# DLR-RM/curvature

Measured on AMD Instinct MI355X. Metric: KFAC factor-build + invert + sample throughput, higher is better.
Workload: dtype f32

## Files before the change

### curvature_amd/_lib.py

```python
import ctypes
import os
import subprocess
import threading

_HERE = os.path.dirname(os.path.abspath(__file__))
CSRC = os.path.join(_HERE, "csrc")
INCLUDE = os.path.normpath(os.path.join(_HERE, "..", "include"))
LIB_PATH = os.path.join(CSRC, "libcurv_hip.so")
SOURCES = ["api.cpp", "collective.cpp", "elementwise.hip", "syrk.hip", "syrk_flat.hip", "syrk_corr.hip", "syrk_pre.hip", "syrk_small.hip", "group_factor.hip", "kfac_half.hip", "convt_factor.hip", "dilated_factor.hip", "conv3d_factor.hip", "reduce_factor.hip", "persample.hip", "persample_dw.hip", "norm_factor.hip", "logit_mc.hip", "head_mc.hip", "head_grid.hip", "invert.hip", "gemm.hip", "inf.hip", "eigh.hip", "eigh_lowrank.hip", "logdet.hip"]
HIPCC_FLAGS = ["-O3", "--offload-arch=gfx950", "-std=c++17", "-fPIC", "-shared", "-Wall",
               "-Wno-unused-function", "-ldl"]

_lock = threading.Lock()
_lib = None


def _stale() -> bool:
    if not os.path.exists(LIB_PATH):
        return True
    t = os.path.getmtime(LIB_PATH)
    deps = [os.path.join(CSRC, f) for f in os.listdir(CSRC) if f.endswith((".hip", ".cpp", ".h"))]
    deps.append(os.path.join(INCLUDE, "curv_hip.h"))
    return any(os.path.getmtime(d) > t for d in deps)


def _compiler_id(hipcc: str) -> str:
    try:
        return subprocess.run([hipcc, "--version"], stdout=subprocess.PIPE, stderr=subprocess.STDOUT, text=True).stdout
    except OSError as exc:
        raise RuntimeError(f"cannot run {hipcc}: {exc}")


def build(force: bool = False, verbose: bool = False) -> str:
    if not force and not _stale():
        return LIB_PATH
    import fcntl
    import hashlib
    from concurrent.futures import ThreadPoolExecutor
    hipcc = os.environ.get("HIPCC", "hipcc")
    objdir = os.path.join(CSRC, "build")
    os.makedirs(objdir, exist_ok=True)
    headers = sorted([os.path.join(CSRC, f) for f in os.listdir(CSRC) if f.endswith(".h")] + [os.path.join(INCLUDE, "curv_hip.h")])
    compile_flags = [f for f in HIPCC_FLAGS if f not in ("-shared", "-ldl")] + ["-c"]
    base = hashlib.sha256()
    base.update(_compiler_id(hipcc).encode())
    base.update(" ".join(compile_flags).encode())
    for h in headers:
        base.update(open(h, "rb").read())

    def compile_one(src):
        path = os.path.join(CSRC, src)
        obj = os.path.join(objdir, src + ".o")
        key = base.copy()
        key.update(open(path, "rb").read())
        stamp, want = obj + ".stamp", key.hexdigest()
        if not force and os.path.exists(obj) and os.path.exists(stamp) and open(stamp).read() == want:
            return obj, 0, ""
        tmp = f"{obj}.{os.getpid()}.tmp"
        cmd = [hipcc] + compile_flags + ["-o", tmp, path]
        if verbose:
            print(" ".join(cmd[:-3] + ["-o", obj, path]), flush=True)
        proc = subprocess.run(cmd, stdout=subprocess.PIPE, stderr=subprocess.STDOUT, text=True)
        if proc.returncode == 0:
            os.replace(tmp, obj)
            with open(stamp + ".tmp", "w") as fh:
                fh.write(want)
            os.replace(stamp + ".tmp", stamp)
        elif os.path.exists(tmp):
            os.remove(tmp)
        return obj, proc.returncode, proc.stdout

    with open(os.path.join(objdir, ".lock"), "w") as lock:
        fcntl.flock(lock, fcntl.LOCK_EX)
        try:
            if not force and not _stale():
                return LIB_PATH
            with ThreadPoolExecutor(max_workers=int(os.environ.get("CURV_BUILD_JOBS", "6"))) as pool:
                results = list(pool.map(compile_one, SOURCES))
            for obj, rc, out in results:
                if rc != 0:
                    raise RuntimeError("hipcc failed:\n" + out)
                if verbose and out:
                    print(out)
            tmp = f"{LIB_PATH}.{os.getpid()}.tmp"
            cmd = [hipcc, "--offload-arch=gfx950", "-fPIC", "-shared", "-o", tmp] + [r[0] for r in results] + ["-ldl"]
            if verbose:
                print(" ".join(cmd), flush=True)
            proc = subprocess.run(cmd, stdout=subprocess.PIPE, stderr=subprocess.STDOUT, text=True)
            if proc.returncode != 0:
                if os.path.exists(tmp):
                    os.remove(tmp)
                raise RuntimeError("hipcc (link) failed:\n" + proc.stdout)
            os.replace(tmp, LIB_PATH)
        finally:
            fcntl.flock(lock, fcntl.LOCK_UN)
    return LIB_PATH


_ENDS = [("src", ctypes.c_void_p), ("dst", ctypes.c_void_p)]
_SOURCE = [(k, ctypes.c_int32) for k in ("N", "C", "H", "W")]
_WINDOW = [(k, ctypes.c_int32) for k in ("kh", "kw", "sh", "sw", "ph", "pw")]
_ENTRY = [("has_bias", ctypes.c_int32), ("first", ctypes.c_int32), ("scale", ctypes.c_float)]


class curv_factor_desc(ctypes.Structure):
    _fields_ = _ENDS + _SOURCE + _WINDOW + _ENTRY + [("path_hint", ctypes.c_int32)]


class curv_group_factor_desc(ctypes.Structure):
    _fields_ = _ENDS + _SOURCE + [("groups", ctypes.c_int32)] + _WINDOW + _ENTRY


class curv_convt_factor_desc(ctypes.Structure):
    _fields_ = _ENDS + _SOURCE + _WINDOW + [("Ho", ctypes.c_int32), ("Wo", ctypes.c_int32)] + _ENTRY


class curv_dilated_factor_desc(ctypes.Structure):
    _fields_ = _ENDS + _SOURCE + _WINDOW + _ENTRY + [("dh", ctypes.c_int32), ("dw", ctypes.c_int32)]


class curv_conv3d_factor_desc(ctypes.Structure):
    _fields_ = _ENDS + [(k, ctypes.c_int32) for k in ("N", "C", "D", "H", "W", "kd", "kh", "kw", "sd", "sh", "sw", "pd", "ph",
                                                     "pw")] + _ENTRY


class curv_reduce_factor_desc(ctypes.Structure):
    _fields_ = _ENDS + _SOURCE + _WINDOW + _ENTRY + [(k, ctypes.c_int32) for k in ("dtype", "form", "mean", "T", "E")]


class curv_factor16_desc(ctypes.Structure):
    _fields_ = _ENDS + _SOURCE + _WINDOW + _ENTRY + [("dtype", ctypes.c_int32)]


class curv_inv_desc(ctypes.Structure):
    _fields_ = [("F", ctypes.c_void_p), ("L", ctypes.c_void_p), ("n", ctypes.c_int32), ("reserved", ctypes.c_int32),
                ("add", ctypes.c_double), ("multiply", ctypes.c_double)]


class curv_gemm_desc(ctypes.Structure):
    _fields_ = [("A", ctypes.c_void_p), ("B", ctypes.c_void_p), ("C", ctypes.c_void_p), ("E", ctypes.c_void_p)] + \
               [(k, ctypes.c_longlong) for k in ("a_rs", "a_cs", "b_rs", "b_cs", "c_rs", "c_cs", "e_rs", "e_cs")] + \
               [("M", ctypes.c_int32), ("N", ctypes.c_int32), ("K", ctypes.c_int32), ("epilogue", ctypes.c_int32),
                ("alpha", ctypes.c_float), ("beta", ctypes.c_float), ("tri", ctypes.c_int32),
                ("reserved", ctypes.c_int32), ("F", ctypes.c_void_p), ("f_rs", ctypes.c_longlong),
                ("f_cs", ctypes.c_longlong)]


class curv_cholinv_desc(ctypes.Structure):
    _fields_ = [("M", ctypes.c_void_p), ("X", ctypes.c_void_p), ("n", ctypes.c_int32), ("m_is_f64", ctypes.c_int32),
                ("diag_add", ctypes.c_double), ("R", ctypes.c_void_p), ("r_minus", ctypes.c_int32), ("reserved", ctypes.c_int32),
                ("pivot_min", ctypes.c_double)]


class curv_gemm64_desc(ctypes.Structure):
    _fields_ = [("A", ctypes.c_void_p), ("B", ctypes.c_void_p), ("C", ctypes.c_void_p)] + \
               [(k, ctypes.c_longlong) for k in ("a_rs", "a_cs", "b_rs", "b_cs", "c_rs", "c_cs")] + \
               [("M", ctypes.c_int32), ("N", ctypes.c_int32), ("K", ctypes.c_int32), ("tri", ctypes.c_int32),
                ("alpha", ctypes.c_double), ("beta", ctypes.c_double),
                ("E", ctypes.c_void_p), ("row_scale", ctypes.c_void_p), ("col_scale", ctypes.c_void_p), ("C32", ctypes.c_void_p)]


class curv_sq_desc(ctypes.Structure):
    _fields_ = [("grad_w", ctypes.c_void_p), ("grad_b", ctypes.c_void_p), ("state", ctypes.c_void_p),
                ("rows", ctypes.c_int32), ("cols_w", ctypes.c_int32), ("first", ctypes.c_int32),
                ("reserved", ctypes.c_int32)]


class curv_persample_desc(ctypes.Structure):
    _fields_ = [("A", ctypes.c_void_p), ("B", ctypes.c_void_p), ("C", ctypes.c_void_p)] + \
               [(k, ctypes.c_longlong) for k in ("a_ns", "a_rs", "b_ns", "b_rs", "c_rs")] + \
               [("S", ctypes.c_int32), ("M", ctypes.c_int32), ("Nc", ctypes.c_int32), ("L", ctypes.c_int32),
                ("first", ctypes.c_int32), ("alpha", ctypes.c_float)]


class curv_persample_quad_desc(ctypes.Structure):
    _fields_ = [("A", ctypes.c_void_p), ("B", ctypes.c_void_p), ("W", ctypes.c_void_p), ("out", ctypes.c_void_p)] + \
               [(k, ctypes.c_longlong) for k in ("a_ns", "a_rs", "b_ns", "b_rs", "w_rs", "o_stride")] + \
               [("S", ctypes.c_int32), ("M", ctypes.c_int32), ("Nc", ctypes.c_int32), ("L", ctypes.c_int32),
                ("first", ctypes.c_int32), ("alpha", ctypes.c_float)]


class curv_persample_project_desc(ctypes.Structure):
    _fields_ = [(k, ctypes.c_void_p) for k in ("A", "B", "W", "U", "Z")] + \
               [(k, ctypes.c_longlong) for k in ("a_ns", "a_rs", "b_ns", "b_rs", "w_rs", "u_rs", "z_ns", "z_rs", "z_cs")] + \
               [(k, ctypes.c_int32) for k in ("S", "M", "Nc", "L", "R", "first")] + \
               [("alpha", ctypes.c_float), ("reserved", ctypes.c_int32)]


class curv_persample_grid_desc(ctypes.Structure):
    _fields_ = [(k, ctypes.c_void_p) for k in ("A", "B", "u", "v", "V", "out")] + \
               [("shift", ctypes.POINTER(ctypes.c_float)), ("gain", ctypes.POINTER(ctypes.c_float))] + \
               [(k, ctypes.c_longlong) for k in ("a_ns", "a_rs", "b_ns", "b_rs", "v_rs", "o_stride", "o_hs")] + \
               [(k, ctypes.c_int32) for k in ("S", "M", "Nc", "L", "H", "first")]


class curv_persample_cov_desc(ctypes.Structure):
    _fields_ = [("A", ctypes.c_void_p), ("B", ctypes.c_void_p), ("W", ctypes.c_void_p), ("out", ctypes.c_void_p)] + \
               [(k, ctypes.c_longlong) for k in ("a_cs", "a_ns", "a_rs", "b_ns", "b_rs", "w_rs", "o_ns", "o_rs")] + \
               [(k, ctypes.c_int32) for k in ("S", "K", "M", "Nc", "L", "first")] + [("alpha", ctypes.c_float)]


class curv_logit_mc_desc(ctypes.Structure):
    _fields_ = [(k, ctypes.c_void_p) for k in ("cov", "mu", "rest", "Z", "probs", "probs_rest", "draws", "info")] + \
               [(k, ctypes.c_longlong) for k in ("o_ns", "o_rs", "mu_ns", "z_ns", "z_ss")] + \
               [("seed", ctypes.c_ulonglong), ("offset", ctypes.c_ulonglong)] + \
               [(k, ctypes.c_int32) for k in ("N", "K", "S", "reserved")]


class curv_head_mc_desc(ctypes.Structure):
    _fields_ = [(k, ctypes.c_void_p) for k in ("M", "d2", "mu", "Z", "probs", "draws")] + \
               [(k, ctypes.c_longlong) for k in ("m_rs", "d_ns", "d_cs", "mu_ns", "z_ns", "z_ss")] + \
               [("seed", ctypes.c_ulonglong), ("offset", ctypes.c_ulonglong)] + \
               [(k, ctypes.c_int32) for k in ("N", "K", "S", "m_lower")] + [("reserved", ctypes.c_longlong)]


class curv_head_moments_desc(ctypes.Structure):
    _fields_ = curv_head_mc_desc._fields_[:-1] + \
               [("entropy", ctypes.c_void_p), ("probs_sq", ctypes.c_void_p), ("reserved", ctypes.c_longlong)]


class curv_head_grid_desc(ctypes.Structure):
    _fields_ = [(k, ctypes.c_void_p) for k in ("Y", "u", "v", "T", "out")] + \
               [("shift", ctypes.POINTER(ctypes.c_float)), ("gain", ctypes.POINTER(ctypes.c_float))] + \
               [(k, ctypes.c_longlong) for k in ("y_rs", "t_rs")] + [(k, ctypes.c_int32) for k in ("N", "K", "n", "H")]


class curv_persample_pack_desc(ctypes.Structure):
    _fields_ = _ENDS + _SOURCE + _WINDOW + \
               [(k, ctypes.c_int32) for k in ("has_bias", "channels_last", "rows_outer", "Lp")]


class curv_persample_pack_ex_desc(ctypes.Structure):
    _fields_ = _ENDS + [(k, ctypes.c_longlong) for k in ("s_n", "s_c", "s_h", "s_w", "src_elems")] + _SOURCE + _WINDOW + \
               [(k, ctypes.c_int32) for k in ("Ho", "Wo", "has_bias", "dtype", "transposed", "rows_outer", "Lp", "reserved")]


class curv_persample_pack3d_desc(ctypes.Structure):
    _fields_ = _ENDS + [(k, ctypes.c_longlong) for k in ("s_n", "s_c", "s_d", "s_h", "s_w", "src_elems")] + \
               [(k, ctypes.c_int32) for k in ("N", "C", "D", "H", "W", "kd", "kh", "kw", "sd", "sh", "sw", "pd", "ph", "pw",
                                              "has_bias", "dtype", "rows_outer", "Lp", "reserved")]


class curv_persample_dw_desc(ctypes.Structure):
    _fields_ = [("x", ctypes.c_void_p), ("g", ctypes.c_void_p)] + \
               [(k, ctypes.c_longlong) for k in ("x_sn", "x_sc", "x_sh", "x_sw", "x_elems",
                                                 "g_sn", "g_sc", "g_sh", "g_sw", "g_elems")] + _SOURCE + _WINDOW + \
               [(k, ctypes.c_int32) for k in ("Ho", "Wo", "has_bias", "first")] + [("alpha", ctypes.c_float),
                                                                                   ("reserved", ctypes.c_int32)] + \
               [("dst", ctypes.c_void_p), ("c_rs", ctypes.c_longlong)] + \
               [(k, ctypes.c_void_p) for k in ("T", "Wt", "s", "out")] + \
               [(k, ctypes.c_longlong) for k in ("t_cs", "t_rs", "w_rs", "o_stride")]


class curv_norm_desc(ctypes.Structure):
    _fields_ = [("x", ctypes.c_void_p), ("g", ctypes.c_void_p)] + \
               [(k, ctypes.c_longlong) for k in ("x_sn", "x_sc", "x_sh", "x_sw", "x_elems",
                                                 "g_sn", "g_sc", "g_sh", "g_sw", "g_elems")] + _SOURCE + \
               [("mode", ctypes.c_int32), ("groups", ctypes.c_int32), ("eps", ctypes.c_float), ("has_bias", ctypes.c_int32),
                ("mean", ctypes.c_void_p), ("var", ctypes.c_void_p), ("side", ctypes.c_int32), ("first", ctypes.c_int32),
                ("scale", ctypes.c_float), ("alpha", ctypes.c_float), ("reserved", ctypes.c_int32),
                ("reserved2", ctypes.c_int32), ("dst", ctypes.c_void_p), ("c_rs", ctypes.c_longlong)] + \
               [(k, ctypes.c_void_p) for k in ("T", "Wt", "s", "out")] + \
               [(k, ctypes.c_longlong) for k in ("t_cs", "t_rs", "w_rs", "o_stride")]


_DW_RECORD = [("x", ctypes.c_void_p), ("g", ctypes.c_void_p)] + \
             [(k, ctypes.c_longlong) for k in ("x_sn", "x_sc", "x_sh", "x_sw", "x_elems",
                                               "g_sn", "g_sc", "g_sh", "g_sw", "g_elems")] + _SOURCE + _WINDOW + \
             [(k, ctypes.c_int32) for k in ("Ho", "Wo", "has_bias")]


class curv_persample_dw_project_desc(ctypes.Structure):
    _fields_ = _DW_RECORD + [("reserved", ctypes.c_int32)] + [(k, ctypes.c_void_p) for k in ("T", "Wt", "s", "y")] + \
               [(k, ctypes.c_longlong) for k in ("t_cs", "t_rs", "w_rs", "y_ns")]


class curv_persample_dw_grid_desc(ctypes.Structure):
    _fields_ = _DW_RECORD + [("first", ctypes.c_int32)] + [(k, ctypes.c_void_p) for k in ("T", "u", "v", "V", "out")] + \
               [("shift", ctypes.POINTER(ctypes.c_float)), ("gain", ctypes.POINTER(ctypes.c_float))] + \
               [(k, ctypes.c_longlong) for k in ("t_cs", "t_rs", "v_rs", "o_stride", "o_hs")] + \
               [("Hn", ctypes.c_int32), ("reserved", ctypes.c_int32)]


class curv_persample_gram_desc(ctypes.Structure):
    _fields_ = [("Y", ctypes.c_void_p), ("out", ctypes.c_void_p)] + \
               [(k, ctypes.c_longlong) for k in ("y_ks", "y_ns", "o_ns", "o_rs")] + \
               [(k, ctypes.c_int32) for k in ("N", "K", "E", "first")] + [("alpha", ctypes.c_float), ("reserved", ctypes.c_int32)]


class curv_copy_desc(ctypes.Structure):
    _fields_ = [("dst", ctypes.c_void_p), ("src", ctypes.c_void_p), ("bytes", ctypes.c_ulonglong)]


class curv_eigh_desc(ctypes.Structure):
    _fields_ = [("F", ctypes.c_void_p), ("U", ctypes.c_void_p), ("w", ctypes.c_void_p), ("n", ctypes.c_int32),
                ("reserved", ctypes.c_int32)]


class curv_logsum_desc(ctypes.Structure):
    _fields_ = [("x", ctypes.c_void_p), ("dtype", ctypes.c_int32), ("mode", ctypes.c_int32), ("count", ctypes.c_int64),
                ("stride", ctypes.c_int64), ("weight", ctypes.c_double), ("gain", ctypes.c_double * 16),
                ("shift", ctypes.c_double * 16)]


class curv_select_desc(ctypes.Structure):
    _fields_ = [("lambda_vec", ctypes.c_void_p), ("I", ctypes.c_void_p), ("J", ctypes.c_void_p),
                ("counts", ctypes.c_void_p), ("n", ctypes.c_int32), ("m", ctypes.c_int32), ("rank", ctypes.c_int32),
                ("reserved", ctypes.c_int32)]


_vp, _i, _ll, _d, _sz = ctypes.c_void_p, ctypes.c_int, ctypes.c_longlong, ctypes.c_double, ctypes.c_size_t

SIGNATURES = {
    "curv_version": (_i, []),
    "curv_last_error": (ctypes.c_char_p, []),
    "curv_init_streams": (_i, []),
    "curv_allgather_weights": (_i, [_vp, _vp, _vp, ctypes.POINTER(ctypes.c_longlong), ctypes.POINTER(ctypes.c_longlong)]),
    "curv_rccl_available": (_i, []),
    "curv_comm_unique_id": (_i, [_vp]),
    "curv_comm_init": (_i, [ctypes.POINTER(_vp), _i, _vp, _i]),
    "curv_comm_destroy": (_i, [_vp]),
    "curv_kfac_workspace_bytes": (_sz, [ctypes.POINTER(curv_factor_desc), _i]),
    "curv_kfac_plan_info": (_i, [ctypes.POINTER(curv_factor_desc), _i, ctypes.POINTER(ctypes.c_longlong)]),
    "curv_kfac_path_for": (_i, [ctypes.POINTER(curv_factor_desc), _i]),
    "curv_kfac_accumulate": (_i, [_vp, ctypes.POINTER(curv_factor_desc), _i, _vp, _sz]),
    "curv_kfac_accumulate_timed": (_i, [_vp, ctypes.POINTER(curv_factor_desc), _i, _vp, _sz, _vp, _vp]),
    "curv_kfac_accumulate_ex": (_i, [_vp, ctypes.POINTER(curv_factor_desc), _i, _vp, _sz, ctypes.c_uint, _vp, _vp]),
    "curv_kfac_group_workspace_bytes": (_sz, [ctypes.POINTER(curv_group_factor_desc), _i]),
    "curv_kfac_group_plan_flops": (_i, [ctypes.POINTER(curv_group_factor_desc), _i, ctypes.POINTER(ctypes.c_longlong)]),
    "curv_kfac_group_accumulate": (_i, [_vp, ctypes.POINTER(curv_group_factor_desc), _i, _vp, _sz]),
    "curv_kfac16_workspace_bytes": (_sz, [ctypes.POINTER(curv_factor16_desc), _i]),
    "curv_kfac16_plan_flops": (_i, [ctypes.POINTER(curv_factor16_desc), _i, ctypes.POINTER(ctypes.c_longlong)]),
    "curv_kfac16_accumulate": (_i, [_vp, ctypes.POINTER(curv_factor16_desc), _i, _vp, _sz]),
    "curv_kfac_convt_workspace_bytes": (_sz, [ctypes.POINTER(curv_convt_factor_desc), _i]),
    "curv_kfac_convt_plan_flops": (_i, [ctypes.POINTER(curv_convt_factor_desc), _i, ctypes.POINTER(ctypes.c_longlong)]),
    "curv_kfac_convt_accumulate": (_i, [_vp, ctypes.POINTER(curv_convt_factor_desc), _i, _vp, _sz]),
    "curv_kfac_dilated_workspace_bytes": (_sz, [ctypes.POINTER(curv_dilated_factor_desc), _i]),
    "curv_kfac_dilated_plan_flops": (_i, [ctypes.POINTER(curv_dilated_factor_desc), _i, ctypes.POINTER(ctypes.c_longlong)]),
    "curv_kfac_dilated_accumulate": (_i, [_vp, ctypes.POINTER(curv_dilated_factor_desc), _i, _vp, _sz]),
    "curv_kfac_conv3d_workspace_bytes": (_sz, [ctypes.POINTER(curv_conv3d_factor_desc), _i]),
    "curv_kfac_conv3d_plan_flops": (_i, [ctypes.POINTER(curv_conv3d_factor_desc), _i, ctypes.POINTER(ctypes.c_longlong)]),
    "curv_kfac_conv3d_accumulate": (_i, [_vp, ctypes.POINTER(curv_conv3d_factor_desc), _i, _vp, _sz]),
    "curv_kfac_reduce_workspace_bytes": (_sz, [ctypes.POINTER(curv_reduce_factor_desc), _i]),
    "curv_kfac_reduce_plan_flops": (_i, [ctypes.POINTER(curv_reduce_factor_desc), _i, ctypes.POINTER(ctypes.c_longlong)]),
    "curv_kfac_reduce_accumulate": (_i, [_vp, ctypes.POINTER(curv_reduce_factor_desc), _i, _vp, _sz]),
    "curv_event_create": (_vp, []),
    "curv_event_destroy": (None, [_vp]),
    "curv_event_elapsed_ms": (_i, [_vp, _vp, ctypes.POINTER(ctypes.c_float)]),
    "curv_event_synchronize": (_i, [_vp]),
    "curv_chol_inv_workspace_bytes": (_sz, [ctypes.POINTER(curv_inv_desc), _i]),
    "curv_chol_inv_lower": (_i, [_vp, ctypes.POINTER(curv_inv_desc), _i, _vp, _vp, _sz]),
    "curv_chol_inv_lower_status": (_i, [_vp, ctypes.POINTER(curv_inv_desc), _i, _vp, _vp, _sz, _vp, _vp]),
    "curv_chol_factor_inverse_workspace_bytes": (_sz, [ctypes.POINTER(curv_cholinv_desc), _i]),
    "curv_chol_factor_inverse": (_i, [_vp, ctypes.POINTER(curv_cholinv_desc), _i, _vp, _vp, _sz]),
    "curv_gemm_f64_batched": (_i, [_vp, ctypes.POINTER(curv_gemm64_desc), _i]),
    "curv_syevd_workspace_bytes": (_sz, [ctypes.POINTER(curv_eigh_desc), _i]),
    "curv_syevd": (_i, [_vp, ctypes.POINTER(curv_eigh_desc), _i, _vp, _sz, _i, _d, ctypes.POINTER(ctypes.c_int)]),
    "curv_syevd_ex": (_i, [_vp, ctypes.POINTER(curv_eigh_desc), _i, _vp, _sz, _i, _d, ctypes.POINTER(ctypes.c_int),
                          ctypes.POINTER(ctypes.c_int)]),
    "curv_inf_select": (_i, [_vp, ctypes.POINTER(curv_select_desc), _i]),
    "curv_colpairs": (_i, [_vp, _vp, _i, _i, _ll, _vp]),
    "curv_inf_vtv_assemble": (_i, [_vp, _vp, _vp, _i, _i, _vp]),
    "curv_inf_vtv_assemble_f64": (_i, [_vp, _vp, _vp, _i, _i, _vp]),
    "curv_colpairs_f64": (_i, [_vp, _vp, _i, _i, _ll, _vp]),
    "curv_colpairs_sym_f64": (_i, [_vp, _vp, _i, _i, _ll, _vp]),
    "curv_inf_vtv_assemble_sym_f64": (_i, [_vp, _vp, _vp, _i, _i, _vp]),
    "curv_square_f64": (_i, [_vp, _vp, _vp, _ll]),
    "curv_diag_scale": (_i, [_vp, _vp, _i, _vp, _vp, _vp, _i, _i]),
    "curv_gather2d": (_i, [_vp, _vp, _ll, _ll, _vp, _vp, _vp, _i, _i]),
    "curv_kron": (_i, [_vp, _vp, _i, _i, _vp, _i, _i, _vp]),
    "curv_mul2d": (_i, [_vp, _vp, _ll, _ll, _vp, _ll, _ll, _vp, _i, _i]),
    "curv_gemm_workspace_bytes": (_sz, [_i]),
    "curv_gemm_workspace_bytes_for": (_sz, [ctypes.POINTER(curv_gemm_desc), _i]),
    "curv_gemm_batched": (_i, [_vp, ctypes.POINTER(curv_gemm_desc), _i, _vp, _sz]),
    "curv_gemm_batched_ex": (_i, [_vp, ctypes.POINTER(curv_gemm_desc), _i, _vp, _sz, ctypes.c_uint]),
    "curv_gemm_plan_info": (_i, [ctypes.POINTER(curv_gemm_desc), _i, _sz, ctypes.POINTER(ctypes.c_longlong)]),
    "curv_randn": (_i, [_vp, _vp, _ll, ctypes.c_ulonglong, ctypes.c_ulonglong]),
    "curv_randn_counter": (_i, [_vp, _vp, ctypes.c_longlong, ctypes.c_ulonglong, _vp]),
    "curv_rsqrt_affine": (_i, [_vp, _vp, _d, _d, _vp, _ll]),
    "curv_sq_accumulate": (_i, [_vp, _vp, _vp, _i, _i, _d, _vp, _i]),
    "curv_sq_accumulate_batched": (_i, [_vp, ctypes.POINTER(curv_sq_desc), _i, _d]),
    "curv_persample_workspace_bytes": (_sz, [ctypes.POINTER(curv_persample_desc), _i]),
    "curv_persample_plan_flops": (_i, [ctypes.POINTER(curv_persample_desc), _i, ctypes.POINTER(ctypes.c_longlong)]),
    "curv_persample_sq_accumulate": (_i, [_vp, ctypes.POINTER(curv_persample_desc), _i, _vp, _sz]),
    "curv_persample_pack": (_i, [_vp, ctypes.POINTER(curv_persample_pack_desc), _i]),
    "curv_persample_pack_ex": (_i, [_vp, ctypes.POINTER(curv_persample_pack_ex_desc), _i]),
    "curv_persample_pack3d": (_i, [_vp, ctypes.POINTER(curv_persample_pack3d_desc), _i]),
    "curv_persample_quad_workspace_bytes": (_sz, [ctypes.POINTER(curv_persample_quad_desc), _i]),
    "curv_persample_quad_plan_flops": (_i, [ctypes.POINTER(curv_persample_quad_desc), _i, ctypes.POINTER(ctypes.c_longlong)]),
    "curv_persample_quad_reduce": (_i, [_vp, ctypes.POINTER(curv_persample_quad_desc), _i, _vp, _sz]),
    "curv_persample_project_workspace_bytes": (_sz, [ctypes.POINTER(curv_persample_project_desc), _i]),
    "curv_persample_project_plan_flops": (_i, [ctypes.POINTER(curv_persample_project_desc), _i, ctypes.POINTER(ctypes.c_longlong)]),
    "curv_persample_project": (_i, [_vp, ctypes.POINTER(curv_persample_project_desc), _i, _vp, _sz]),
    "curv_persample_quad_grid_workspace_bytes": (_sz, [ctypes.POINTER(curv_persample_grid_desc), _i]),
    "curv_persample_quad_grid_plan_flops": (_i, [ctypes.POINTER(curv_persample_grid_desc), _i, ctypes.POINTER(ctypes.c_longlong)]),
    "curv_persample_quad_grid_reduce": (_i, [_vp, ctypes.POINTER(curv_persample_grid_desc), _i, _vp, _sz]),
    "curv_persample_cov_workspace_bytes": (_sz, [ctypes.POINTER(curv_persample_cov_desc), _i]),
    "curv_persample_cov_plan_flops": (_i, [ctypes.POINTER(curv_persample_cov_desc), _i, ctypes.POINTER(ctypes.c_longlong)]),
    "curv_persample_cov_reduce": (_i, [_vp, ctypes.POINTER(curv_persample_cov_desc), _i, _vp, _sz]),
    "curv_persample_dw_workspace_bytes": (_sz, [ctypes.POINTER(curv_persample_dw_desc), _i]),
    "curv_persample_dw_plan_info": (_i, [ctypes.POINTER(curv_persample_dw_desc), _i, ctypes.POINTER(ctypes.c_longlong),
                                        ctypes.POINTER(ctypes.c_longlong)]),
    "curv_persample_dw_sq_accumulate": (_i, [_vp, ctypes.POINTER(curv_persample_dw_desc), _i, _vp, _sz]),
    "curv_persample_dw_quad_reduce": (_i, [_vp, ctypes.POINTER(curv_persample_dw_desc), _i, _vp, _sz]),
    "curv_persample_dw_project_workspace_bytes": (_sz, [ctypes.POINTER(curv_persample_dw_project_desc), _i]),
    "curv_persample_dw_project_plan_info": (_i, [ctypes.POINTER(curv_persample_dw_project_desc), _i,
                                                ctypes.POINTER(ctypes.c_longlong), ctypes.POINTER(ctypes.c_longlong)]),
    "curv_persample_dw_project": (_i, [_vp, ctypes.POINTER(curv_persample_dw_project_desc), _i, _vp, _sz]),
    "curv_persample_dw_quad_grid_workspace_bytes": (_sz, [ctypes.POINTER(curv_persample_dw_grid_desc), _i]),
    "curv_persample_dw_quad_grid_plan_info": (_i, [ctypes.POINTER(curv_persample_dw_grid_desc), _i,
                                                  ctypes.POINTER(ctypes.c_longlong), ctypes.POINTER(ctypes.c_longlong)]),
    "curv_persample_dw_quad_grid_reduce": (_i, [_vp, ctypes.POINTER(curv_persample_dw_grid_desc), _i, _vp, _sz]),
    "curv_kfac_norm_workspace_bytes": (_sz, [ctypes.POINTER(curv_norm_desc), _i]),
    "curv_kfac_norm_plan_flops": (_i, [ctypes.POINTER(curv_norm_desc), _i, ctypes.POINTER(ctypes.c_longlong)]),
    "curv_kfac_norm_accumulate": (_i, [_vp, ctypes.POINTER(curv_norm_desc), _i, _vp, _sz]),
    "curv_persample_norm_workspace_bytes": (_sz, [ctypes.POINTER(curv_norm_desc), _i]),
    "curv_persample_norm_plan_info": (_i, [ctypes.POINTER(curv_norm_desc), _i, ctypes.POINTER(ctypes.c_longlong),
                                          ctypes.POINTER(ctypes.c_longlong)]),
    "curv_persample_norm_sq_accumulate": (_i, [_vp, ctypes.POINTER(curv_norm_desc), _i, _vp, _sz]),
    "curv_persample_norm_quad_reduce": (_i, [_vp, ctypes.POINTER(curv_norm_desc), _i, _vp, _sz]),
    "curv_persample_gram_reduce": (_i, [_vp, ctypes.POINTER(curv_persample_gram_desc), _i]),
    "curv_logit_mc_workspace_bytes": (_sz, [ctypes.POINTER(curv_logit_mc_desc), _i]),
    "curv_logit_mc_plan_flops": (_i, [ctypes.POINTER(curv_logit_mc_desc), _i, ctypes.POINTER(ctypes.c_longlong)]),
    "curv_logit_mc": (_i, [_vp, ctypes.POINTER(curv_logit_mc_desc), _i, _vp, _sz]),
    "curv_head_mc_workspace_bytes": (_sz, [ctypes.POINTER(curv_head_mc_desc), _i]),
    "curv_head_mc_plan_flops": (_i, [ctypes.POINTER(curv_head_mc_desc), _i, ctypes.POINTER(ctypes.c_longlong)]),
    "curv_head_mc": (_i, [_vp, ctypes.POINTER(curv_head_mc_desc), _i, _vp, _sz]),
    "curv_head_mc_moments_workspace_bytes": (_sz, [ctypes.POINTER(curv_head_moments_desc), _i]),
    "curv_head_mc_moments_plan_flops": (_i, [ctypes.POINTER(curv_head_moments_desc), _i,
                                             ctypes.POINTER(ctypes.c_longlong)]),
    "curv_head_mc_moments": (_i, [_vp, ctypes.POINTER(curv_head_moments_desc), _i, _vp, _sz]),
    "curv_head_grid_workspace_bytes": (_sz, [ctypes.POINTER(curv_head_grid_desc), _i]),
    "curv_head_grid_plan_flops": (_i, [ctypes.POINTER(curv_head_grid_desc), _i, ctypes.POINTER(ctypes.c_longlong)]),
    "curv_head_grid": (_i, [_vp, ctypes.POINTER(curv_head_grid_desc), _i, _vp, _sz]),
    "curv_clamp_min0": (_i, [_vp, _vp, _ll]),
    "curv_sqrt_scale": (_i, [_vp, _vp, _d, _vp, _ll]),
    "curv_mul": (_i, [_vp, _vp, _vp, _vp, _ll]),
    "curv_copy_batched": (_i, [_vp, ctypes.POINTER(curv_copy_desc), _i]),
    "curv_logsum_workspace_bytes": (_sz, [ctypes.POINTER(curv_logsum_desc), _i, _i]),
    "curv_logsum_grid": (_i, [_vp, ctypes.POINTER(curv_logsum_desc), _i, _i, _vp, _ll, _vp, _vp, _sz]),
}


ABI_VERSION = 12
DTYPE_F32, DTYPE_BF16, DTYPE_F16 = 0, 1, 2
KFAC_TABLE_RESIDENT = 1
PATH_AUTO, PATH_SMALL, PATH_GROUPED = 0, 1, 2
REDUCE_PLANE, REDUCE_TOKEN = 0, 1
SMALL_MAX_FLOP = 2.0e9
CONVT_MAX_PHASES = 64
PERSAMPLE_COV_MAX_OUTPUTS = 16
HEAD_MC_MAX_CLASSES = 1024
HEAD_GRID_MAX = 16
PERSAMPLE_GRID_MAX = 16
DTYPE_F64 = 3
LOGSUM_GRID_MAX, LOGSUM_CHUNK, LOGSUM_ROW_BYTES = 16, 4096, 304
LOGSUM_LOG, LOGSUM_SQUARES = 0, 1
NORM_GROUP, NORM_POSITION, NORM_GIVEN = 0, 1, 2
NORM_SIDE_A, NORM_SIDE_G = 0, 1
NORM_SPLIT_L, NORM_SLICE = 1024, 32
GEMM_TABLE_RESIDENT = 1
GEMM_PLAN_FIELDS = 8
ERR_NOT_PD, ERR_INVALID, ERR_WORKSPACE, ERR_HIP, ERR_NOT_CONVERGED = 1, 2, 3, 4, 5


def lib() -> ctypes.CDLL:
    global _lib
    if _lib is not None:
        return _lib
    with _lock:
        if _lib is not None:
            return _lib
        import torch
        if not os.path.exists(LIB_PATH):
            raise RuntimeError(
                f"{LIB_PATH} is missing: run `python -c 'import __graft_entry__ as g; g.build()'` "
                "(hipcc --offload-arch=gfx950). There is no CPU fallback.")
        handle = ctypes.CDLL(LIB_PATH, mode=ctypes.RTLD_GLOBAL)
        for name, (res, args) in SIGNATURES.items():
            fn = getattr(handle, name)
            fn.restype = res
            fn.argtypes = args
        if handle.curv_version() != ABI_VERSION:
            raise RuntimeError("libcurv_hip.so ABI version mismatch")
        _lib = handle
    return _lib


def check(status: int, what: str = "") -> None:
    if status != 0:
        msg = lib().curv_last_error().decode("utf-8", "replace")
        raise RuntimeError(f"libcurv_hip {what} failed with status {status}: {msg}")


def init_streams(device) -> None:
    import torch
    device = torch.device(device)
    if device.type != "cuda":
        return
    with torch.cuda.device(device):
        torch.zeros(1, device=device).add_(1)
        torch.cuda.current_stream(device).synchronize()
        check(lib().curv_init_streams(), "curv_init_streams")


def stream_ptr() -> int:
    import torch
    return int(torch.cuda.current_stream().cuda_stream)
```

### curvature_amd/csrc/invert.hip

```cpp
#include <type_traits>
#include "kernarg.h"
#include "mma64.h"
#include <hip/hip_ext.h>

#include <algorithm>
#include <chrono>
#include <cstdlib>
#include <mutex>
#include <vector>

namespace curv {

constexpr int INV_THREADS = MMA_THREADS;
constexpr int SQ_FLAGS = 32;
constexpr int SQ_FD = 0, SQ_FLC = 4, SQ_FLROW = 8, SQ_FT = 12;
constexpr int SQ_SPIN_LIMIT = 1 << 21;
#ifdef CURV_SQ_TRACE
__device__ long long g_sq_trace[256];
#define KT_BEGIN(slot) { if (threadIdx.x == 0 && k0 == 4 * (CURV_SQ_TRACE - 1)) atomicMax((unsigned long long*)&g_sq_trace[slot], (1ull << 62) - (unsigned long long)wall_clock64()); }
#define KT_END(slot) { if (threadIdx.x == 0 && k0 == 4 * (CURV_SQ_TRACE - 1)) atomicMax((unsigned long long*)&g_sq_trace[slot], (unsigned long long)wall_clock64()); }
#define SQT(slot) { if (threadIdx.x == 0 && f == 0 && stamp == CURV_SQ_TRACE) g_sq_trace[slot] = wall_clock64(); }
#define FIT(k) { if (threadIdx.x == 0 && trace_base >= 0) g_sq_trace[trace_base + (k)] = wall_clock64(); }
#else
#define SQT(slot)
#define FIT(k)
#define KT_BEGIN(slot) {}
#define KT_END(slot) {}
#endif
#ifdef CURV_SQ_TRACE
#define PQT(slot) { if (threadIdx.x == 0 && blockIdx.x == 0 && k0 == 4 * (CURV_SQ_TRACE - 1)) g_sq_trace[slot] = wall_clock64(); }
#else
#define PQT(slot)
#endif

struct InvDev {
  const float* F;
  float* L;
  double* W;
  double* X;
  int* info;
  int n, np, P;
  float sqrt_s, sqrt_n;
  int reverse;
  int f64_in;
  int r_minus;
  double* Xout;
  const double* R;
  double* Zm;
  double add64;
  float* C32;
  float* X32;
  float* S32;
  double pivot_min;
};
typedef __attribute__((address_space(1))) float gfloat;
__device__ __host__ __forceinline__ bool s_in_sweep(const InvDev& d) { return d.X32 == nullptr; }
__device__ __host__ __forceinline__ int s_kind(const InvDev& d) { return d.X32 != nullptr ? 0 : (d.Zm != nullptr ? 2 : 1); }

template <typename CountFn>
__device__ __forceinline__ bool locate(const InvDev* __restrict__ t, int nf, int bid, CountFn cnt, int& f,
                                       int& local) {
  const int lane = threadIdx.x & 63;
  int base = 0;
  for (int f0 = 0; f0 < nf; f0 += 64) {
    const int ff = f0 + lane;
    const int c = (ff < nf) ? cnt(t[ff]) : 0;
    int incl = c;
#pragma unroll
    for (int o = 1; o < 64; o <<= 1) {
      const int v = __shfl_up(incl, o, 64);
      if (lane >= o) incl += v;
    }
    const int total = __builtin_amdgcn_readfirstlane(__shfl(incl, 63, 64));
    if (bid < base + total) {
      const unsigned long long m = __ballot(bid < base + incl);
      const int l = __ffsll((long long)m) - 1;
      f = __builtin_amdgcn_readfirstlane(f0 + l);
      local = __builtin_amdgcn_readfirstlane(bid - (base + __shfl(incl - c, l, 64)));
      return true;
    }
    base += total;
  }
  return false;
}

__global__ void __launch_bounds__(INV_THREADS)
inv_prepare_kernel(const InvDev* __restrict__ t, int nf, int* __restrict__ flags) {
  int f, tile;
  if (!locate(t, nf, blockIdx.x, [](const InvDev& d) { return d.P * (d.P + 1) / 2; }, f, tile)) return;
  const InvDev& d = t[f];
  int bi = 0;
  while (tile > bi) { tile -= bi + 1; ++bi; }
  const int bj = tile;
  const int n = d.n, np = d.np, rev = d.reverse;
  const float ss = d.sqrt_s, sn = d.sqrt_n;
  const gfloat* F = (const gfloat*)d.F;
  gdouble* W = (gdouble*)d.W;
  if (bi == 0 && bj == 0 && threadIdx.x == 0) *d.info = 0;
  if (bi == 0 && bj == 0 && threadIdx.x < SQ_FLAGS) flags[(long long)f * SQ_FLAGS + threadIdx.x] = 0;
  if (d.Zm != nullptr) {
    const gdouble* Rg = (const gdouble*)d.R;
    gdouble* Z = (gdouble*)d.Zm;
    const int w0 = __builtin_amdgcn_readfirstlane(threadIdx.x >> 6), c0 = threadIdx.x & 63;
    const int jj = bj * NB + c0;
#pragma unroll 4
    for (int u = 0; u < 16; ++u) {
      const int i = bi * NB + w0 + 4 * u;
      Z[(long long)i * np + jj] = (i < n && jj <= i) ? Rg[(long long)i * n + jj] : 0.0;
    }
  }
  if (d.f64_in) {
    const gdouble* M = (const gdouble*)d.F;
    const int w0 = __builtin_amdgcn_readfirstlane(threadIdx.x >> 6), c0 = threadIdx.x & 63;
    const int jj = bj * NB + c0;
#pragma unroll 4
    for (int u = 0; u < 16; ++u) {
      const int i = bi * NB + w0 + 4 * u;
      double v;
      if (i < n && jj < n) {
        v = 0.5 * (M[(long long)i * n + jj] + M[(long long)jj * n + i]);
        if (i == jj) v += d.add64;
      } else {
        v = (i == jj) ? 1.0 : 0.0;
      }
      W[(long long)i * np + jj] = v;
    }
    return;
  }
  __shared__ float Tm[NB][NB + 1];
  const int w = __builtin_amdgcn_readfirstlane(threadIdx.x >> 6), c = threadIdx.x & 63;
  const int j = bj * NB + c, rj = rev ? n - 1 - j : j;
  const int mi = bi * NB + c, rmi = rev ? n - 1 - mi : mi;
  float fd[16], fm[16];
#pragma unroll
  for (int u = 0; u < 16; ++u) {
    const int r = w + 4 * u;
    const int i = bi * NB + r, ri = rev ? n - 1 - i : i;
    const int mj = bj * NB + r, rmj = rev ? n - 1 - mj : mj;
    fd[u] = (i < n && j < n) ? F[(long long)ri * n + rj] : 0.0f;
    fm[u] = (mi < n && mj < n) ? F[(long long)rmj * n + rmi] : 0.0f;
  }
#pragma unroll
  for (int u = 0; u < 16; ++u) Tm[w + 4 * u][c] = fm[u];
  __syncthreads();
#pragma unroll
  for (int u = 0; u < 16; ++u) {
    const int r = w + 4 * u;
    const int i = bi * NB + r;
    double v;
    if (i < n && j < n) {
      float a = __fmul_rn(ss, fd[u]);
      float b = __fmul_rn(ss, Tm[c][r]);
      if (i == j) { a = __fadd_rn(a, sn); b = __fadd_rn(b, sn); }
      v = (double)__fmul_rn(__fadd_rn(a, b), 0.5f);
    } else {
      v = (i == j) ? 1.0 : 0.0;
    }
    W[(long long)i * np + j] = v;
  }
}

__device__ __host__ __forceinline__ long long inner_tiles(int P, int k, int k0, int kend) {
  const int ke = kend < P ? kend : P;
  long long tr = 0;
  for (int j = k + 1; j < ke; ++j) tr += ke - j;
  const long long sr = (ke - k - 1 > 0) ? (long long)(ke - k - 1) * (k - k0 + 1) : 0;
  return tr + sr;
}
constexpr int SB = 4;
__device__ __host__ __forceinline__ long long outer_tiles(int P, int kend, int row0, bool s_part) {
  const long long r = P - row0;
  if (r <= 0) return 0;
  const long long nsb = (r + SB - 1) / SB, ncb = s_part ? (kend + SB - 1) / SB : 0;
  return (nsb * (nsb + 1) / 2 + nsb * ncb) * (SB * SB);
}
__device__ __host__ __forceinline__ long long strip_tiles(int P, int kend, int lo, int hi, bool s_part) {
  const int re = hi < P ? hi : P;
  long long n = 0;
  for (int j = lo; j < re; ++j) n += P - j;
  if (s_part && re > lo) n += (long long)(re - lo) * kend;
  return n;
}

__device__ __forceinline__ void store_sub(gdouble* C, int np, const f64x4 (&acc)[2][2], int wm, int wn, int lane,
                                          int mode) {
  store_acc(C, np, acc, wm, wn, lane, mode);
}

__device__ __forceinline__ void factor_invert_64(double* Ds, double* Is, int* bad, int pivot_base, double pivot_min, int trace_base = -1);
__device__ __forceinline__ void lds_sub_acc(double* s, const f64x4 (&acc)[2][2], int wm, int wn, int lane);

__global__ void __launch_bounds__(INV_THREADS)
inner_update_kernel(const InvDev* __restrict__ t, int nf, int k, int k0, int kend) {
  __shared__ double As[NB * LDA], Bs[NB * LDA];
  int f, local;
  if (!locate(t, nf, blockIdx.x, [k, k0, kend](const InvDev& d) { return (int)inner_tiles(d.P, k, k0, kend); }, f, local)) return;
  const InvDev& d = t[f];
  const int np = d.np, P = d.P, ke = kend < P ? kend : P;
  gdouble* W = (gdouble*)d.W;
  gdouble* X = (gdouble*)d.X;
  const int lane = threadIdx.x & 63, wave = threadIdx.x >> 6, wm = wave >> 1, wn = wave & 1;
  f64x4 acc[2][2] = {};
  int j = k + 1;
  bool trailing = false;
  for (; j < ke; ++j) {
    if (local < ke - j) { trailing = true; break; }
    local -= ke - j;
  }
  if (trailing) {
    const int i = j + local;
    load_block(W + (long long)i * NB * np + k * NB, np, As);
    if (i != j) load_block(W + (long long)j * NB * np + k * NB, np, Bs);
    __syncthreads();
    mma_64<true>(As, (i != j) ? Bs : As, wm, wn, lane, acc);
    if (i == j && j == k + 1) {
      __shared__ int bad;
      __syncthreads();
      if (threadIdx.x == 0) bad = 0;
      load_block(W + (long long)j * NB * np + j * NB, np, As);
      __syncthreads();
      {
        const int c16 = lane & 15, rq = lane >> 4;
#pragma unroll
        for (int m = 0; m < 2; ++m)
#pragma unroll
          for (int n = 0; n < 2; ++n)
#pragma unroll
            for (int q = 0; q < 4; ++q)
              As[(32 * wm + 16 * m + rq + 4 * q) * LDA + 32 * wn + 16 * n + c16] -= acc[m][n][q];
      }
      __syncthreads();
      factor_invert_64(As, Bs, &bad, j * NB, d.pivot_min);
      store_block(X + (long long)j * NB * np + j * NB, np, Bs);
      if (threadIdx.x == 0 && bad != 0) atomicCAS(d.info, 0, bad);
    } else {
      store_sub(W + (long long)i * NB * np + j * NB, np, acc, wm, wn, lane, 0);
    }
  } else {
    const int w = k - k0 + 1;
    const int a = local / w, jj = k0 + local - a * w;
    const int i = k + 1 + a;
    load_block(W + (long long)i * NB * np + k * NB, np, As);
    load_block(X + (long long)k * NB * np + jj * NB, np, Bs);
    __syncthreads();
    mma_64<false>(As, Bs, wm, wn, lane, acc);
    store_sub(X + (long long)i * NB * np + jj * NB, np, acc, wm, wn, lane, jj == k ? 1 : 2);
  }
}

constexpr int OKS = 16;
constexpr int OPA = OKS + 1;
struct TileJob {
  const gbyte* a0;
  const gbyte* b0;
  gdouble* C;
  int np, ke0, ke1, mode;
  bool bt, same;
  gfloat* C32 = nullptr;
};
__device__ __forceinline__ void store_acc_f32(gfloat* __restrict__ C, int ld, const f64x4 (&acc)[2][2], int wm, int wn, int lane,
                                              float sign) {
  const int c16 = lane & 15, rq = lane >> 4;
  const unsigned voff = (unsigned)(((long long)(32 * wm + rq) * ld + 32 * wn + c16) * 4);
  gbyte* base = (gbyte*)C;
#pragma unroll
  for (int m = 0; m < 2; ++m)
#pragma unroll
    for (int n = 0; n < 2; ++n)
#pragma unroll
      for (int q = 0; q < 4; ++q)
        *(gfloat*)(base + ((long long)(16 * m + 4 * q) * ld + 16 * n) * 4 + voff) = sign * (float)acc[m][n][q];
}
template <int WV, int MODE>
__device__ __forceinline__ void tile_product_impl(const TileJob& o, double* __restrict__ As, double* __restrict__ Bs) {
  constexpr int THREADS = 64 * WV * WV, T = 4 / WV, LPT = NB * OKS / THREADS;
  const int np = o.np;
  const int tid = threadIdx.x, lane = tid & 63, wave = tid >> 6, wm = wave / WV, wn = wave % WV;
  constexpr bool trailing = MODE != 2, same = MODE == 1;
  const int r16 = lane & 15, kq = lane >> 4;
  double ra[LPT], rb[LPT];
  const unsigned voff_k = (unsigned)(((long long)(tid / OKS) * np + (tid % OKS)) * 8);
  constexpr int BE = 8;
  const unsigned voff_n = (unsigned)(((long long)(tid >> 6) * np + (tid & 63)) * BE);
  const long long step_k = (long long)(THREADS / OKS) * np * 8, step_n = (long long)(THREADS / 64) * np * BE;
  auto fetch = [&](int ke) __attribute__((always_inline)) {
    const gbyte* ga = o.a0 + (long long)ke * 8;
    const gbyte* gb = trailing ? o.b0 + (long long)ke * 8 : o.b0 + (long long)ke * np * BE;
#pragma unroll
    for (int u = 0; u < LPT; ++u) {
      ra[u] = *(const gdouble*)(ga + u * step_k + voff_k);
      if (trailing) rb[u] = same ? 0.0 : *(const gdouble*)(gb + u * step_k + voff_k);
      else rb[u] = *(const gdouble*)(gb + u * step_n + voff_n);
    }
  };
  f64x4 acc[T][T] = {};
  const int ke0 = o.ke0, ke1 = o.ke1;
  fetch(ke0);
  for (int ke = ke0; ke < ke1; ke += OKS) {
#pragma unroll
    for (int u = 0; u < LPT; ++u) {
      const int e = tid + u * THREADS;
      As[(e / OKS) * OPA + (e % OKS)] = ra[u];
      if (trailing) { if (!same) Bs[(e / OKS) * OPA + (e % OKS)] = rb[u]; }
      else Bs[(e >> 6) * LDA + (e & 63)] = rb[u];
    }
    __syncthreads();
    if (ke + OKS < ke1) fetch(ke + OKS);
    const double* Bt = same ? As : Bs;
#pragma unroll 4
    for (int ks = 0; ks < OKS / 4; ++ks) {
      const int k = 4 * ks + kq;
      double a[T], b[T];
#pragma unroll
      for (int m = 0; m < T; ++m) a[m] = As[(16 * T * wm + 16 * m + r16) * OPA + k];
#pragma unroll
      for (int n = 0; n < T; ++n)
        b[n] = trailing ? Bt[(16 * T * wn + 16 * n + r16) * OPA + k] : Bs[k * LDA + 16 * T * wn + 16 * n + r16];
#pragma unroll
      for (int m = 0; m < T; ++m)
#pragma unroll
        for (int n = 0; n < T; ++n) acc[m][n] = __builtin_amdgcn_mfma_f64_16x16x4f64(a[m], b[n], acc[m][n], 0, 0, 0);
    }
    __syncthreads();
  }
  if constexpr (WV == 2) {
    store_acc(o.C, np, acc, wm, wn, lane, o.mode);
    if (o.C32 != nullptr) store_acc_f32(o.C32, np, acc, wm, wn, lane, 1.0f);
  } else {
    const int c16 = lane & 15, rq = lane >> 4;
    if (o.C32 != nullptr) {
      gbyte* b32 = (gbyte*)o.C32;
      const unsigned v32 = (unsigned)(((long long)(16 * wm + rq) * np + 16 * wn + c16) * 4);
#pragma unroll
      for (int q = 0; q < 4; ++q) *(gfloat*)(b32 + (long long)(4 * q) * np * 4 + v32) = (float)acc[0][0][q];
    }
    gbyte* base = (gbyte*)o.C;
    const unsigned voff = (unsigned)(((long long)(16 * wm + rq) * np + 16 * wn + c16) * 8);
    double old[4];
    if (o.mode == 0 || o.mode == 2) {
#pragma unroll
      for (int q = 0; q < 4; ++q) old[q] = *(const gdouble*)(base + (long long)(4 * q) * np * 8 + voff);
    }
#pragma unroll
    for (int q = 0; q < 4; ++q) {
      const double v = acc[0][0][q];
      const double out = o.mode == 0 ? old[q] - v : o.mode == 1 ? v : o.mode == 2 ? old[q] + v : -v;
      *(gdouble*)(base + (long long)(4 * q) * np * 8 + voff) = out;
    }
  }
}

template <int WV>
__device__ __forceinline__ void tile_product_k32(const TileJob& o, double* __restrict__ As, double* __restrict__ Bs) {
  if (!o.bt) tile_product_impl<WV, 2>(o, As, Bs);
  else if (o.same) tile_product_impl<WV, 1>(o, As, Bs);
  else tile_product_impl<WV, 0>(o, As, Bs);
}

template <int WV>
__device__ __forceinline__ void outer_update_body(const InvDev* __restrict__ t, int nf, int k0, int kend, int lo, int hi,
                                                  int strip, int n_items, double* __restrict__ As, double* __restrict__ Bs) {
  bool trailing;
  int i, j, f, local;
  if (strip == 1) {
    if (!locate(t, nf, blockIdx.x, [kend, lo, hi](const InvDev& d) { return (int)strip_tiles(d.P, kend, lo, hi, s_in_sweep(d)); }, f, local))
      return;
    const int P = t[f].P, re = hi < P ? hi : P;
    trailing = false;
    j = lo;
    for (; j < re; ++j) {
      if (local < P - j) { trailing = true; break; }
      local -= P - j;
    }
    if (trailing) {
      i = j + local;
    } else {
      const int a = local / kend;
      i = lo + a; j = local - a * kend;
    }
  } else {
    const int row0 = lo;
    int item;
    {
      const int bid = blockIdx.x, xcd = bid & 7, jj = bid >> 3;
      item = ((jj / (SB * SB)) * 8 + xcd) * (SB * SB) + (jj % (SB * SB));
    }
    if (item >= n_items) return;
    if (!locate(t, nf, item, [kend, row0](const InvDev& d) {
          return (int)(outer_tiles(d.P, kend, row0, s_in_sweep(d)) - outer_tiles(d.P, kend, row0, false)); }, f, local)) return;
    const int r = t[f].P - row0;
    const int s2 = local / (SB * SB), in = local % (SB * SB);
    const int di = in / SB, dj = in - di * SB;
    const int ncb = (kend + SB - 1) / SB;
    const int a = s2 / ncb, cb = s2 - a * ncb;
    const int ri = a * SB + di; j = cb * SB + dj;
    if (ri >= r || j >= kend) return;
    trailing = false; i = row0 + ri;
  }
  const InvDev& d = t[f];
  const int np = d.np;
  const gdouble* W = (const gdouble*)d.W;
  gdouble* X = (gdouble*)d.X;
  TileJob o;
  o.np = np;
  o.bt = trailing;
  o.same = trailing && i == j;
  o.a0 = (const gbyte*)(W + (long long)i * NB * np);
  gdouble* Sx = d.Zm != nullptr ? (gdouble*)d.Zm : X;
  o.b0 = trailing ? (const gbyte*)(W + (long long)j * NB * np) : (const gbyte*)(Sx + j * NB);
  o.ke0 = (trailing ? k0 : (j > k0 ? j : k0)) * NB;
  o.ke1 = kend * NB;
  o.C = trailing ? (gdouble*)d.W + (long long)i * NB * np + j * NB : Sx + (long long)i * NB * np + j * NB;
  o.mode = trailing ? 0 : (d.Zm != nullptr ? 0 : (j >= k0 ? 1 : 2));
  tile_product_k32<WV>(o, As, Bs);
}
__global__ void __launch_bounds__(INV_THREADS, 3)
outer_update_kernel(const InvDev* __restrict__ t, int nf, int k0, int kend, int lo, int hi, int strip, int n_items) {
  __shared__ double As[NB * OPA], Bs[NB * OPA > OKS * LDA ? NB * OPA : OKS * LDA];
  outer_update_body<2>(t, nf, k0, kend, lo, hi, strip, n_items, As, Bs);
}
typedef __attribute__((address_space(3))) void lds_void;
typedef __attribute__((address_space(3))) char lds_char;
typedef double f64x2 __attribute__((ext_vector_type(2)));
namespace fard {
constexpr int ROW_B = 128, TILE_B = NB * ROW_B, KS = 16;
}
__global__ void __launch_bounds__(INV_THREADS, 4)
outer_update_dma_kernel(const InvDev* __restrict__ t, int nf, int k0, int kend, int row0, int n_items) {
  using namespace fard;
  __shared__ __attribute__((aligned(1024))) char smem[4 * TILE_B];
  lds_char* lds = (lds_char*)smem;
  int item;
  {
    const int bid = blockIdx.x, xcd = bid & 7, jj = bid >> 3;
    item = ((jj / (SB * SB)) * 8 + xcd) * (SB * SB) + (jj % (SB * SB));
  }
  if (item >= n_items) return;
  int f, local;
  if (!locate(t, nf, item, [kend, row0](const InvDev& d) { return (int)outer_tiles(d.P, kend, row0, false); }, f, local)) return;
  const InvDev& d = t[f];
  int i, j;
  {
    const int r = d.P - row0;
    const int sb = local / (SB * SB), in = local - sb * (SB * SB);
    const int di = in / SB, dj = in - di * SB;
    int a = 0, tl = sb;
    while (tl > a) { tl -= a + 1; ++a; }
    const int ri = a * SB + di, rj = tl * SB + dj;
    if (ri >= r || rj > ri) return;
    i = row0 + ri; j = row0 + rj;
  }
  const int np = d.np;
  const int tid = threadIdx.x, lane = tid & 63;
  const int wave = __builtin_amdgcn_readfirstlane(tid >> 6), wm = wave >> 1, wn = wave & 1;
  const int r16 = lane & 15, kq = lane >> 4;
  const bool same = i == j;
  const unsigned panel_b = (unsigned)((long long)NB * np * 8);
  const __amdgpu_buffer_rsrc_t rs_a =
      __builtin_amdgcn_make_buffer_rsrc((void*)(d.W + (long long)i * NB * np), 0, panel_b, 0x00020000);
  const __amdgpu_buffer_rsrc_t rs_b =
      __builtin_amdgcn_make_buffer_rsrc((void*)(d.W + (long long)j * NB * np), 0, panel_b, 0x00020000);
  const int drow = 8 * wave + (lane >> 3);
  const int voff = (drow * np) * 8 + (((lane & 7) ^ ((drow >> 1) & 7)) << 4);
  const int half_b = 32 * np * 8;
  auto issue = [&](int ke, unsigned buf) {
    const int kb = ke * 8;
    __builtin_amdgcn_raw_ptr_buffer_load_lds(rs_a, (lds_void*)(lds + buf + wave * 1024), 16, voff, kb, 0, 0);
    __builtin_amdgcn_raw_ptr_buffer_load_lds(rs_a, (lds_void*)(lds + buf + (wave + 4) * 1024), 16, voff, half_b + kb, 0, 0);
    if (!same) {
      __builtin_amdgcn_raw_ptr_buffer_load_lds(rs_b, (lds_void*)(lds + 2 * TILE_B + buf + wave * 1024), 16, voff, kb, 0, 0);
      __builtin_amdgcn_raw_ptr_buffer_load_lds(rs_b, (lds_void*)(lds + 2 * TILE_B + buf + (wave + 4) * 1024), 16, voff, half_b + kb, 0, 0);
    }
  };
  unsigned addr_a[2], addr_b[2];
#pragma unroll
  for (int m = 0; m < 2; ++m) {
    const int ra = 32 * wm + 16 * m + r16, rb = 32 * wn + 16 * m + r16;
    addr_a[m] = ra * ROW_B + ((kq ^ ((ra >> 1) & 7)) << 4);
    addr_b[m] = (same ? 0 : 2 * TILE_B) + rb * ROW_B + ((kq ^ ((rb >> 1) & 7)) << 4);
  }
  f64x4 acc[2][2] = {};
  const int ke0 = k0 * NB, n_st = (kend - k0) * NB / KS;
  issue(ke0, 0);
  for (int st = 0; st < n_st; ++st) {
    __builtin_amdgcn_s_waitcnt(0x0f70);
    __syncthreads();
    const unsigned buf = (st & 1) * TILE_B;
    if (st + 1 < n_st) issue(ke0 + KS * (st + 1), TILE_B - buf);
    f64x2 av[2][2], bv[2][2];
#pragma unroll
    for (int h = 0; h < 2; ++h)
#pragma unroll
      for (int m = 0; m < 2; ++m) {
        av[m][h] = *reinterpret_cast<const __attribute__((address_space(3))) f64x2*>(lds + buf + (addr_a[m] ^ (h << 6)));
        bv[m][h] = *reinterpret_cast<const __attribute__((address_space(3))) f64x2*>(lds + buf + (addr_b[m] ^ (h << 6)));
      }
#pragma unroll
    for (int h = 0; h < 2; ++h)
#pragma unroll
      for (int dd = 0; dd < 2; ++dd)
#pragma unroll
        for (int m = 0; m < 2; ++m)
#pragma unroll
          for (int n = 0; n < 2; ++n) acc[m][n] = __builtin_amdgcn_mfma_f64_16x16x4f64(av[m][h][dd], bv[n][h][dd], acc[m][n], 0, 0, 0);
  }
  store_acc((gdouble*)d.W + (long long)i * NB * np + j * NB, np, acc, wm, wn, lane, 0);
}

__global__ void __launch_bounds__(1024)
outer_update_wide_kernel(const InvDev* __restrict__ t, int nf, int k0, int kend, int lo, int hi, int strip, int n_items) {
  __shared__ double As[NB * OPA], Bs[NB * OPA > OKS * LDA ? NB * OPA : OKS * LDA];
  KT_BEGIN(252)
  outer_update_body<4>(t, nf, k0, kend, lo, hi, strip, n_items, As, Bs);
  KT_END(253)
}

__device__ __forceinline__ double readlane_f64(double v, int src_lane) {
  const int lo = __builtin_amdgcn_readlane(__double2loint(v), src_lane);
  const int hi = __builtin_amdgcn_readlane(__double2hiint(v), src_lane);
  return __hiloint2double(hi, lo);
}

template <bool BT>
__device__ __forceinline__ void mma16(const double* Ap, int lda, const double* Bp, int ldb, int lane, f64x4& acc) {
  const int r16 = lane & 15, kq = lane >> 4;
#pragma unroll
  for (int ks = 0; ks < 4; ++ks) {
    const int kk = 4 * ks + kq;
    const double a = Ap[r16 * lda + kk];
    const double b = BT ? Bp[r16 * ldb + kk] : Bp[kk * ldb + r16];
    acc = __builtin_amdgcn_mfma_f64_16x16x4f64(a, b, acc, 0, 0, 0);
  }
}

__device__ __forceinline__ double rsqrt_pos(double x) {
  double y = __builtin_amdgcn_rsq(x);
  const double hx = 0.5 * x;
  y = y * fma(-hx * y, y, 1.5);
  y = y * fma(-hx * y, y, 1.5);
  return y;
}

__device__ __forceinline__ double rcp_pos(double x) {
  const double y = __builtin_amdgcn_rcp(x);
  const double e = fma(-x, y, 1.0);
  return fma(y, fma(e, e, e), y);
}

__device__ __forceinline__ void factor_invert_64(double* Ds, double* Is, int* bad, int pivot_base, double pivot_min, int trace_base) {
  (void)trace_base;
  __shared__ double Sc[4][16 * 17];
  __shared__ double dinv_s[NB];
  const int tid = threadIdx.x, lane = tid & 63, wave = tid >> 6;
  const int r16 = lane & 15, kq = lane >> 4;
  auto diag_inverse = [&](int b) {
    if (lane < 16) {
      const double* Lb = Ds + 16 * b * LDA + 16 * b;
      double x[16], sum[16], col[16], dv[16];
#pragma unroll
      for (int r = 0; r < 16; ++r) { sum[r] = 0.0; col[r] = r > 0 ? Lb[r * LDA] : 0.0; dv[r] = dinv_s[16 * b + r]; }
#pragma unroll
      for (int q = 0; q < 16; ++q) {
        x[q] = ((q == lane ? 1.0 : 0.0) - sum[q]) * dv[q];
        double nxt[16];
#pragma unroll
        for (int r = q + 2; r < 16; ++r) nxt[r] = Lb[r * LDA + q + 1];
#pragma unroll
        for (int r = q + 1; r < 16; ++r) sum[r] += col[r] * x[q];
#pragma unroll
        for (int r = q + 2; r < 16; ++r) col[r] = nxt[r];
      }
#pragma unroll
      for (int r = 0; r < 16; ++r) Is[(16 * b + r) * LDA + 16 * b + lane] = x[r];
    }
  };
  auto wave_sync = [&]() {
    __builtin_amdgcn_fence(__ATOMIC_RELEASE, "wavefront");
    __builtin_amdgcn_wave_barrier();
    __builtin_amdgcn_fence(__ATOMIC_ACQUIRE, "wavefront");
  };
  auto block_sum = [&](int i, int b, int k_lo, int k_hi, f64x4& acc) {
    for (int kk = k_lo; kk < k_hi; ++kk)
      mma16<false>(Ds + 16 * i * LDA + 16 * kk, LDA, Is + 16 * kk * LDA + 16 * b, LDA, lane, acc);
  };
  auto finish_block = [&](int i, int b, const f64x4& acc) {
#pragma unroll
    for (int r = 0; r < 4; ++r) Sc[wave][(kq + 4 * r) * 17 + r16] = acc[r];
    wave_sync();
    f64x4 out = {0.0, 0.0, 0.0, 0.0};
    mma16<false>(Is + 16 * i * LDA + 16 * i, LDA, Sc[wave], 17, lane, out);
#pragma unroll
    for (int r = 0; r < 4; ++r) Is[(16 * i + kq + 4 * r) * LDA + 16 * b + r16] = -out[r];
  };
  f64x4 y3 = {0.0, 0.0, 0.0, 0.0};
  const int b3 = wave == 2 ? 0 : wave == 3 ? 1 : 2;
#ifndef CURV_FI_UNROLL
#define CURV_FI_UNROLL 4
#endif
#pragma unroll CURV_FI_UNROLL
  for (int p = 0; p < 4; ++p) {
    const int c0 = 16 * p;
    if (wave != 0) {
      if (p == 0) {
        for (int e = tid - 64; e < NB * NB; e += MMA_THREADS - 64) Is[(e >> 6) * LDA + (e & 63)] = 0.0;
      } else if (wave == 1) {
        diag_inverse(p - 1);
        wave_sync();
        for (int b = 0; b < p - 1; ++b) {
          f64x4 acc = {0.0, 0.0, 0.0, 0.0};
          block_sum(p - 1, b, b, p - 1, acc);
          finish_block(p - 1, b, acc);
          wave_sync();
        }
      } else if (p == 3) {
        block_sum(3, b3, b3, 2, y3);
      }
    }
    if (wave == 0) {
      double row[16];
      int mine_lo = 0, mine_hi = 0x3ff00000;
#pragma unroll
      for (int c = 0; c < 16; ++c) row[c] = Ds[lane * LDA + c0 + c];
      double d = readlane_f64(row[0], c0), rd = rcp_pos(d);
      auto column = [&](auto cc) {
        constexpr int c = decltype(cc)::value;
        asm("v_writelane_b32 %0, %1, %2" : "+v"(mine_lo) : "s"(__double2loint(d)), "n"(c));
        asm("v_writelane_b32 %0, %1, %2" : "+v"(mine_hi) : "s"(__double2hiint(d)), "n"(c));
        if (c + 1 < 16) {
          const double pv = fma(-(row[c] * row[c]), rd, row[c + 1 < 16 ? c + 1 : c]);
          d = readlane_f64(pv, c0 + c + 1);
        }
        const double t = row[c] * rd;
        if (c + 1 < 16) rd = rcp_pos(d);
        double m_next = c + 1 < 16 ? readlane_f64(t, c0 + c + 1) : 0.0;
#pragma unroll
        for (int q = c + 1; q < 16; ++q) {
          const double m = m_next;
          if (q + 1 < 16) m_next = readlane_f64(t, c0 + q + 1);
          row[q] -= row[c] * m;
        }
        __builtin_amdgcn_sched_barrier(0);
      };
#define CURV_COL(C) column(std::integral_constant<int, C>{});
      CURV_COL(0) CURV_COL(1) CURV_COL(2) CURV_COL(3) CURV_COL(4) CURV_COL(5) CURV_COL(6) CURV_COL(7)
      CURV_COL(8) CURV_COL(9) CURV_COL(10) CURV_COL(11) CURV_COL(12) CURV_COL(13) CURV_COL(14) CURV_COL(15)
#undef CURV_COL
      const double mine = __hiloint2double(mine_hi, mine_lo);
      const unsigned long long failed = __ballot(lane < 16 && !(mine > pivot_min && mine < 1.0e300));
      const int first_bad = failed != 0 ? pivot_base + c0 + __ffsll((long long)failed) : 0;
      const double rs = rsqrt_pos(lane < 16 ? mine : 1.0);
      if (lane < 16) dinv_s[c0 + lane] = rs;
      wave_sync();
#pragma unroll
      for (int c = 0; c < 16; ++c) Ds[lane * LDA + c0 + c] = row[c] * dinv_s[c0 + c];
      if (first_bad != 0 && lane == 0 && *bad == 0) *bad = first_bad;
    }
    __syncthreads();
    {
      int tcount = 0;
      for (int ti = p + 1; ti < 4; ++ti)
        for (int tj = p + 1; tj <= ti; ++tj, ++tcount) {
          if ((tcount & 3) != wave) continue;
          f64x4 acc = {0.0, 0.0, 0.0, 0.0};
          mma16<true>(Ds + 16 * ti * LDA + c0, LDA, Ds + 16 * tj * LDA + c0, LDA, lane, acc);
          double* C = Ds + 16 * ti * LDA + 16 * tj;
#pragma unroll
          for (int r = 0; r < 4; ++r) C[(kq + 4 * r) * LDA + r16] -= acc[r];
        }
    }
    __syncthreads();
    FIT(p)
  }
  if (wave == 0) {
    diag_inverse(3);
  } else {
    block_sum(3, b3, 2, 3, y3);
#pragma unroll
    for (int r = 0; r < 4; ++r) Sc[wave][(kq + 4 * r) * 17 + r16] = y3[r];
  }
  __syncthreads();
  if (wave != 0) {
    f64x4 out = {0.0, 0.0, 0.0, 0.0};
    mma16<false>(Is + 16 * 3 * LDA + 16 * 3, LDA, Sc[wave], 17, lane, out);
#pragma unroll
    for (int r = 0; r < 4; ++r) Is[(16 * 3 + kq + 4 * r) * LDA + 16 * b3 + r16] = -out[r];
  }
  __syncthreads();
}

__global__ void __launch_bounds__(INV_THREADS)
chol_diag_kernel(const InvDev* __restrict__ t, int nf, int k) {
  __shared__ double Ds[NB * LDA];
  __shared__ double Is[NB * LDA];
  __shared__ int bad;
  int f, local;
  if (!locate(t, nf, blockIdx.x, [k](const InvDev& d) { return d.P > k ? 1 : 0; }, f, local)) return;
  const InvDev& d = t[f];
  const int np = d.np, tid = threadIdx.x;
  gdouble* W = (gdouble*)d.W;
  if (tid == 0) bad = 0;
  load_block(W + (long long)k * NB * np + k * NB, np, Ds);
  __syncthreads();
  factor_invert_64(Ds, Is, &bad, k * NB, d.pivot_min);
  store_block((gdouble*)d.X + (long long)k * NB * np + k * NB, np, Is);
  if (tid == 0 && bad != 0) atomicCAS(d.info, 0, bad);
}

__global__ void __launch_bounds__(INV_THREADS)
chol_panel_kernel(const InvDev* __restrict__ t, int nf, int k, int k0, int kend) {
  __shared__ double As[NB * LDA], Bs[NB * LDA];
  int f, local;
  if (!locate(t, nf, blockIdx.x,
              [k, k0, kend](const InvDev& d) { return d.P > k ? (kend < d.P ? kend : d.P) - k0 - 1 : 0; }, f, local))
    return;
  const InvDev& d = t[f];
  const int np = d.np, n_solve = (kend < d.P ? kend : d.P) - k - 1;
  gdouble* W = (gdouble*)d.W;
  gdouble* X = (gdouble*)d.X;
  const int lane = threadIdx.x & 63, wave = threadIdx.x >> 6, wm = wave >> 1, wn = wave & 1;
  f64x4 acc[2][2] = {};
  if (local < n_solve) {
    const int i = k + 1 + local;
    load_block(W + (long long)i * NB * np + k * NB, np, As);
    load_block(X + (long long)k * NB * np + k * NB, np, Bs);
    __syncthreads();
    mma_64<true>(As, Bs, wm, wn, lane, acc);
    store_acc(W + (long long)i * NB * np + k * NB, np, acc, wm, wn, lane, 1);
  } else {
    const int j = k0 + local - n_solve;
    load_block(X + (long long)k * NB * np + k * NB, np, As);
    load_block(X + (long long)k * NB * np + j * NB, np, Bs);
    __syncthreads();
    mma_64<false>(As, Bs, wm, wn, lane, acc);
    store_acc(X + (long long)k * NB * np + j * NB, np, acc, wm, wn, lane, 3);
  }
}


__device__ __forceinline__ void load_block_coh(const gdouble* __restrict__ g, int ld, double* __restrict__ s) {
  const int tid = threadIdx.x, r0 = tid >> 6, c = tid & 63;
  const long long step = 4ll * ld;
  const double* base = (const double*)g + (long long)r0 * ld + c;
  double v[NB * NB / MMA_THREADS];
#pragma unroll
  for (int u = 0; u < NB * NB / MMA_THREADS; ++u)
    v[u] = __hip_atomic_load(base + u * step, __ATOMIC_RELAXED, __HIP_MEMORY_SCOPE_AGENT);
#pragma unroll
  for (int u = 0; u < NB * NB / MMA_THREADS; ++u) s[(r0 + 4 * u) * LDA + c] = v[u];
}
__device__ __forceinline__ void store_block_coh(gdouble* __restrict__ g, int ld, const double* __restrict__ s) {
  const int tid = threadIdx.x, r0 = tid >> 6, c = tid & 63;
  const long long step = 4ll * ld;
  double* base = (double*)g + (long long)r0 * ld + c;
#pragma unroll
  for (int u = 0; u < NB * NB / MMA_THREADS; ++u)
    __hip_atomic_store(base + u * step, s[(r0 + 4 * u) * LDA + c], __ATOMIC_RELAXED, __HIP_MEMORY_SCOPE_AGENT);
}
__device__ __forceinline__ void store_acc_coh(gdouble* __restrict__ C, int ld, const f64x4 (&acc)[2][2], int wm, int wn,
                                              int lane, double sign) {
  const int c16 = lane & 15, rq = lane >> 4;
  double* base = (double*)C + (long long)(32 * wm + rq) * ld + 32 * wn + c16;
#pragma unroll
  for (int m = 0; m < 2; ++m)
#pragma unroll
    for (int n = 0; n < 2; ++n)
#pragma unroll
      for (int q = 0; q < 4; ++q)
        __hip_atomic_store(base + (long long)(16 * m + 4 * q) * ld + 16 * n, sign * acc[m][n][q], __ATOMIC_RELAXED,
                           __HIP_MEMORY_SCOPE_AGENT);
}
__device__ __forceinline__ void lds_sub_acc(double* s, const f64x4 (&acc)[2][2], int wm, int wn, int lane) {
  const int c16 = lane & 15, rq = lane >> 4;
#pragma unroll
  for (int m = 0; m < 2; ++m)
#pragma unroll
    for (int n = 0; n < 2; ++n)
#pragma unroll
      for (int q = 0; q < 4; ++q) s[(32 * wm + 16 * m + rq + 4 * q) * LDA + 32 * wn + 16 * n + c16] -= acc[m][n][q];
}
template <bool BT>
__device__ __forceinline__ void mma_64_pre(const double* __restrict__ As, const double* __restrict__ Bs, int wm, int wn, int lane,
                                           f64x4 (&acc)[2][2]) {
  const int r16 = lane & 15, kq = lane >> 4;
  double a[2][16], b[2][16];
#pragma unroll
  for (int m = 0; m < 2; ++m)
#pragma unroll
    for (int ks = 0; ks < 16; ++ks) a[m][ks] = As[(32 * wm + 16 * m + r16) * LDA + 16 * kq + ks];
#pragma unroll
  for (int n = 0; n < 2; ++n)
#pragma unroll
    for (int ks = 0; ks < 16; ++ks)
      b[n][ks] = BT ? Bs[(32 * wn + 16 * n + r16) * LDA + 16 * kq + ks] : Bs[(16 * kq + ks) * LDA + 32 * wn + 16 * n + r16];
#pragma unroll
  for (int ks = 0; ks < 16; ++ks)
#pragma unroll
    for (int m = 0; m < 2; ++m)
#pragma unroll
      for (int n = 0; n < 2; ++n) acc[m][n] = __builtin_amdgcn_mfma_f64_16x16x4f64(a[m][ks], b[n][ks], acc[m][n], 0, 0, 0);
}
__device__ __forceinline__ void zero_acc(f64x4 (&acc)[2][2]) {
#pragma unroll
  for (int m = 0; m < 2; ++m)
#pragma unroll
    for (int n = 0; n < 2; ++n) acc[m][n] = f64x4{0.0, 0.0, 0.0, 0.0};
}
__device__ __forceinline__ void sq_signal(int* flag, int stamp) {
  asm volatile("s_waitcnt vmcnt(0)" ::: "memory");
  __syncthreads();
  if (threadIdx.x == 0) __hip_atomic_store(flag, stamp, __ATOMIC_RELAXED, __HIP_MEMORY_SCOPE_AGENT);
}
__device__ __forceinline__ void sq_wait(int* flag, int stamp, int* lost) {
  if (threadIdx.x == 0) {
    int n = 0;
    while (__hip_atomic_load(flag, __ATOMIC_RELAXED, __HIP_MEMORY_SCOPE_AGENT) < stamp) {
      __builtin_amdgcn_s_sleep(2);
      if (++n > SQ_SPIN_LIMIT || *lost) { *lost = 1; break; }
    }
  }
  __syncthreads();
}

__global__ void __launch_bounds__(INV_THREADS)
chol_square_kernel(const InvDev* __restrict__ t, int nf, int k0, int kend, int* __restrict__ flags, int stamp) {
  __shared__ double Ds[NB * LDA], Is[NB * LDA], Bf[NB * LDA];
  __shared__ int bad, lost;
  int f, r;
  if (!locate(t, nf, blockIdx.x, [k0, kend](const InvDev& d) { return d.P > k0 ? (kend < d.P ? kend : d.P) - k0 : 0; }, f, r))
    return;
  const InvDev& d = t[f];
  const int np = d.np, tid = threadIdx.x;
  const int nbf = (kend < d.P ? kend : d.P) - k0;
  gdouble* W = (gdouble*)d.W;
  gdouble* X = (gdouble*)d.X;
  int* fl = flags + (long long)f * SQ_FLAGS;
  const int lane = tid & 63, wave = tid >> 6, wm = wave >> 1, wn = wave & 1;
  auto Wt = [&](int i, int j) { return W + (long long)(k0 + i) * NB * np + (k0 + j) * NB; };
  auto Xt = [&](int i, int j) { return X + (long long)(k0 + i) * NB * np + (k0 + j) * NB; };
  if (tid == 0) { bad = 0; lost = 0; }
  __syncthreads();
  f64x4 acc[2][2];
  if (r == 0) {
    SQT(0)
#ifdef CURV_SQ_TRACE
    if (tid == 0 && f == 0 && stamp == CURV_SQ_TRACE + 1) g_sq_trace[238] = wall_clock64();
#endif
    load_block(Wt(0, 0), np, Ds);
    if (nbf > 1) load_block(Wt(1, 0), np, Bf);
    __syncthreads();
    SQT(1)
    for (int q = 0; q < nbf; ++q) {
      if (q >= 1) {
        if (q >= 2) {
          sq_wait(fl + SQ_FT + q, stamp, &lost);
          SQT(8 * q + 0)
          load_block_coh(Wt(q, q - 1), np, Bf);
        }
        load_block_coh(Wt(q, q), np, Ds);
        __syncthreads();
        SQT(8 * q + 1)
        zero_acc(acc);
        mma_64_pre<true>(Bf, Is, wm, wn, lane, acc);
        SQT(8 * q + 2)
        store_acc_coh(Wt(q, q - 1), np, acc, wm, wn, lane, 1.0);
        __syncthreads();
        acc_to_lds(acc, wm, wn, lane, Bf);
        __syncthreads();
        zero_acc(acc);
        mma_64_pre<true>(Bf, Bf, wm, wn, lane, acc);
        lds_sub_acc(Ds, acc, wm, wn, lane);
        SQT(8 * q + 3)
        sq_signal(fl + SQ_FLC + q, stamp);
        SQT(8 * q + 4)
      }
#ifdef CURV_SQ_TRACE
      factor_invert_64(Ds, Is, &bad, (k0 + q) * NB, d.pivot_min, (f == 0 && stamp == CURV_SQ_TRACE) ? 112 + 4 * q : -1);
#else
      factor_invert_64(Ds, Is, &bad, (k0 + q) * NB, d.pivot_min);
#endif
      SQT(q == 0 ? 2 : 8 * q + 5)
      store_block_coh(Xt(q, q), np, Is);
      sq_signal(fl + SQ_FD + q, stamp);
      SQT(q == 0 ? 3 : 8 * q + 6)
    }
    if (tid == 0 && bad != 0) atomicCAS(d.info, 0, bad);
    if (tid == 0 && lost != 0) atomicCAS(d.info, 0, -1);
    return;
  }
  double* Af = Ds;
  SQT(64 * r + 0)
  double* Cf = Is;
  if (r >= 2) {
    f64x4 accA[2][2], accT0[2][2], accT1[2][2];
    zero_acc(accA); zero_acc(accT0); zero_acc(accT1);
    auto push = [&](int mp, int m) {
      load_block_coh(Wt(mp, m), np, Bf);
      __syncthreads();
      if (mp == 1) mma_64_pre<true>(Cf, Bf, wm, wn, lane, accT0);
      else mma_64_pre<true>(Cf, Bf, wm, wn, lane, accT1);
      __syncthreads();
    };
    for (int m = 0; m <= r - 2; ++m) {
      SQT(64 * r + 8 + 4 * m)
      load_block(Wt(r, m), np, Af);
      __syncthreads();
      if (m == 1) lds_sub_acc(Af, accT0, wm, wn, lane);
      sq_wait(fl + SQ_FD + m, stamp, &lost);
      SQT(64 * r + 9 + 4 * m)
      load_block_coh(Xt(m, m), np, Bf);
      __syncthreads();
      zero_acc(acc);
      mma_64_pre<true>(Af, Bf, wm, wn, lane, acc);
      SQT(64 * r + 10 + 4 * m)
      store_acc_coh(Wt(r, m), np, acc, wm, wn, lane, 1.0);
      acc_to_lds(acc, wm, wn, lane, Cf);
      if (m == r - 2) sq_signal(fl + SQ_FLROW + r, stamp);
      else __syncthreads();
      mma_64_pre<true>(Cf, Cf, wm, wn, lane, accA);
      __syncthreads();
      for (int mp = m + 1; mp <= r - 1; ++mp) {
        if (m == r - 2 && mp == r - 1) break;
        sq_wait(fl + (mp == m + 1 ? SQ_FLC : SQ_FLROW) + mp, stamp, &lost);
        push(mp, m);
      }
    }
    load_block(Wt(r, r), np, Bf);
    __syncthreads();
    lds_sub_acc(Bf, accA, wm, wn, lane);
    __syncthreads();
    store_block_coh(Wt(r, r), np, Bf);
    load_block(Wt(r, r - 1), np, Af);
    sq_wait(fl + SQ_FLC + r - 1, stamp, &lost);
    push(r - 1, r - 2);
    if (r == 2) lds_sub_acc(Af, accT0, wm, wn, lane);
    else lds_sub_acc(Af, accT1, wm, wn, lane);
    __syncthreads();
    store_block_coh(Wt(r, r - 1), np, Af);
    sq_signal(fl + SQ_FT + r, stamp);
    SQT(64 * r + 1)
  }
  {
    const int j = r - 1;
    for (int i = r; i < nbf; ++i) {
      f64x4 S[2][2];
      zero_acc(S);
      for (int m = j; m < i; ++m) {
        if (m == i - 1) sq_wait(fl + SQ_FLC + i, stamp, &lost);
        else sq_wait(fl + SQ_FLROW + i, stamp, &lost);
        if (m == j) sq_wait(fl + SQ_FD + j, stamp, &lost);
        load_block_coh(Wt(i, m), np, Af);
        load_block_coh(Xt(m, j), np, Bf);
        __syncthreads();
        mma_64_pre<false>(Af, Bf, wm, wn, lane, S);
        __syncthreads();
      }
      SQT(64 * r + 2 + 16 * (i - r))
      acc_to_lds(S, wm, wn, lane, Af);
      sq_wait(fl + SQ_FD + i, stamp, &lost);
      SQT(64 * r + 3 + 16 * (i - r))
      load_block_coh(Xt(i, i), np, Bf);
      __syncthreads();
      zero_acc(acc);
      mma_64_pre<false>(Bf, Af, wm, wn, lane, acc);
      store_acc_coh(Xt(i, j), np, acc, wm, wn, lane, -1.0);
      asm volatile("s_waitcnt vmcnt(0)" ::: "memory");
      __syncthreads();
      SQT(64 * r + 4 + 16 * (i - r))
    }
  }
  if (tid == 0 && lost != 0) atomicCAS(d.info, 0, -1);
}

__device__ __host__ __forceinline__ int panel_jobs(int P, int kind, int k0, int kend) {
  if (P <= k0) return 0;
  return (P > kend ? P - kend : 0) + (kind == 2 ? (kend < P ? kend : P) : kind == 1 ? k0 : 0);
}
template <int WV>
__device__ __forceinline__ void panel_product_body(const InvDev* __restrict__ t, int nf, int k0, int kend,
                                                   double* __restrict__ As, double* __restrict__ Bs) {
  int f, local;
  if (!locate(t, nf, blockIdx.x, [k0, kend](const InvDev& d) { return panel_jobs(d.P, s_kind(d), k0, kend); }, f, local))
    return;
  const InvDev& d = t[f];
  const int np = d.np, nb = (kend < d.P ? kend : d.P) - k0;
  gdouble* W = (gdouble*)d.W;
  gdouble* X = (gdouble*)d.X;
  TileJob o;
  o.np = np;
  o.same = false;
  o.ke0 = 0;
  const int n_below = d.P > kend ? d.P - kend : 0;
  const bool below = local < n_below;
  const int i = kend + local, j = local - n_below;
  o.bt = below;
  o.mode = below ? 1 : 3;
  gdouble* Zm = (gdouble*)d.Zm;
  const bool rhs = !below && Zm != nullptr;
  gdouble* S = rhs ? Zm : X;
  if (rhs) { o.mode = 1; o.ke0 = (j > k0 ? j - k0 : 0) * NB; }
  gfloat* C32 = below ? (gfloat*)d.C32 : nullptr;
  for (int c = nb - 1; c >= 0; --c) {
    if (rhs && k0 + c < j) break;
    const gdouble* xsq = X + (long long)(k0 + c) * NB * np + k0 * NB;
    o.a0 = below ? (const gbyte*)(W + (long long)i * NB * np + k0 * NB) : (const gbyte*)xsq;
    o.b0 = below ? (const gbyte*)xsq : (const gbyte*)(S + (long long)k0 * NB * np + j * NB);
    o.C = below ? W + (long long)i * NB * np + (k0 + c) * NB : S + (long long)(k0 + c) * NB * np + j * NB;
    o.C32 = C32 != nullptr ? C32 + (long long)i * NB * np + (k0 + c) * NB : nullptr;
    o.ke1 = (c + 1) * NB;
    tile_product_k32<WV>(o, As, Bs);
  }
}

constexpr int PQ_PITCH = 4 * NB + 1;
constexpr int PQ_OWN = 16 * PQ_PITCH > 4 * NB * 17 ? 16 * PQ_PITCH : 4 * NB * 17;
template <bool below>
__device__ __forceinline__ void panel_quarter_body(const InvDev& d, int k0, int nb, int i, int j, int q,
                                                   double* __restrict__ Own, double* __restrict__ Ts) {
  const int np = d.np;
  const int tid = threadIdx.x, lane = tid & 63, wave = tid >> 6, r16 = lane & 15, kq = lane >> 4;
  PQT(240)
  const gbyte* Wb = (const gbyte*)d.W;
  const gbyte* Xb = (const gbyte*)d.X;
  if (below) {
    const gbyte* g = Wb + (((long long)i * NB + 16 * q) * np + (long long)k0 * NB) * 8;
    for (int v = 0; v < nb; ++v) {
      double x[4];
#pragma unroll
      for (int u = 0; u < 4; ++u) x[u] = *(const gdouble*)(g + ((long long)((tid >> 6) + 4 * u) * np + (tid & 63) + 64 * v) * 8);
#pragma unroll
      for (int u = 0; u < 4; ++u) Own[((tid >> 6) + 4 * u) * PQ_PITCH + (tid & 63) + 64 * v] = x[u];
    }
  } else {
    const gbyte* g = Xb + ((long long)k0 * NB * np + (long long)j * NB + 16 * q) * 8;
    for (int v = 0; v < nb; ++v) {
      double x[4];
#pragma unroll
      for (int u = 0; u < 4; ++u) {
        x[u] = *(const gdouble*)(g + ((long long)((tid >> 4) + 16 * u + 64 * v) * np + (tid & 15)) * 8);
      }
#pragma unroll
      for (int u = 0; u < 4; ++u) Own[((tid >> 4) + 16 * u + 64 * v) * 17 + (tid & 15)] = x[u];
    }
  }
  double rt0[16], rt1[16], rt2[16];
  auto fetch = [&](int c, int kb, double (&rt)[16]) __attribute__((always_inline)) {
    const gbyte* g = Xb + (((long long)(k0 + c) * NB) * np + (long long)(k0 + kb) * NB) * 8;
#pragma unroll
    for (int u = 0; u < 16; ++u) rt[u] = *(const gdouble*)(g + ((long long)((tid >> 6) + 4 * u) * np + (tid & 63)) * 8);
  };
  auto next = [](int& c, int& kb) { if (++kb > c) { --c; kb = 0; } };
  int c = nb - 1, kb = 0;
  int cf = c, kf = kb;
  fetch(cf, kf, rt0); next(cf, kf);
  if (cf >= 0) { fetch(cf, kf, rt1); next(cf, kf); }
  if (cf >= 0) { fetch(cf, kf, rt2); next(cf, kf); }
  f64x4 acc[4] = {};
  PQT(241)
  [[maybe_unused]] int pq_n = 0;
  auto step = [&](double (&rt)[16]) __attribute__((always_inline)) {
    __syncthreads();
#pragma unroll
    for (int u = 0; u < 16; ++u) Ts[((tid >> 6) + 4 * u) * LDA + (tid & 63)] = rt[u];
    __syncthreads();
    if (cf >= 0) { fetch(cf, kf, rt); next(cf, kf); }
#pragma unroll
    for (int ks = 0; ks < NB / 4; ++ks) {
      const int k = 4 * ks + kq;
      const double a = below ? Own[r16 * PQ_PITCH + 64 * kb + k] : Ts[(16 * wave + r16) * LDA + k];
      const double b = below ? Ts[(16 * wave + r16) * LDA + k] : Own[(64 * kb + k) * 17 + r16];
      acc[ks & 3] = __builtin_amdgcn_mfma_f64_16x16x4f64(a, b, acc[ks & 3], 0, 0, 0);
    }
    if (kb == c) {
      const int wm = below ? q : wave, wn = below ? wave : q;
      const int c16 = lane & 15, rq = lane >> 4;
      gbyte* base = below ? (gbyte*)d.W + (((long long)i * NB) * np + (long long)(k0 + c) * NB) * 8
                          : (gbyte*)d.X + (((long long)(k0 + c) * NB) * np + (long long)j * NB) * 8;
      const unsigned voff = (unsigned)(((long long)(16 * wm + rq) * np + 16 * wn + c16) * 8);
      gbyte* base32 = (below && d.C32 != nullptr) ? (gbyte*)d.C32 + (((long long)i * NB) * np + (long long)(k0 + c) * NB) * 4 : nullptr;
      const unsigned voff32 = (unsigned)(((long long)(16 * wm + rq) * np + 16 * wn + c16) * 4);
#pragma unroll
      for (int qq = 0; qq < 4; ++qq) {
        const double v = (acc[0][qq] + acc[1][qq]) + (acc[2][qq] + acc[3][qq]);
        *(gdouble*)(base + (long long)(4 * qq) * np * 8 + voff) = below ? v : -v;
        if (below && base32 != nullptr) *(gfloat*)(base32 + (long long)(4 * qq) * np * 4 + voff32) = (float)v;
      }
#pragma unroll
      for (int u = 0; u < 4; ++u) acc[u] = f64x4{0.0, 0.0, 0.0, 0.0};
    }
    next(c, kb);
    PQT(242 + pq_n)
    ++pq_n;
  };
  while (c >= 0) {
    step(rt0);
    if (c < 0) break;
    step(rt1);
    if (c < 0) break;
    step(rt2);
  }
}
__global__ void __launch_bounds__(INV_THREADS)
panel_product_quarter_kernel(const InvDev* __restrict__ t, int nf, int k0, int kend) {
  __shared__ double Own[PQ_OWN], Ts[NB * LDA];
  const int job = (blockIdx.x >> 5) * 8 + (blockIdx.x & 7), q = (blockIdx.x >> 3) & 3;
  int f, local;
  KT_BEGIN(236)
  if (!locate(t, nf, job, [k0, kend](const InvDev& d) { return panel_jobs(d.P, s_kind(d), k0, kend); }, f, local)) return;
  const InvDev& d = t[f];
  const int nb = (kend < d.P ? kend : d.P) - k0;
  const int n_below = d.P > kend ? d.P - kend : 0;
  if (local < n_below) panel_quarter_body<true>(d, k0, nb, kend + local, 0, q, Own, Ts);
  else panel_quarter_body<false>(d, k0, nb, 0, local - n_below, q, Own, Ts);
  KT_END(237)
}
__global__ void __launch_bounds__(INV_THREADS, 3)
panel_product_kernel(const InvDev* __restrict__ t, int nf, int k0, int kend) {
  __shared__ double As[NB * OPA], Bs[NB * OPA > OKS * LDA ? NB * OPA : OKS * LDA];
  panel_product_body<2>(t, nf, k0, kend, As, Bs);
}
__global__ void __launch_bounds__(1024)
panel_product_wide_kernel(const InvDev* __restrict__ t, int nf, int k0, int kend) {
  __shared__ double As[NB * OPA], Bs[NB * OPA > OKS * LDA ? NB * OPA : OKS * LDA];
  panel_product_body<4>(t, nf, k0, kend, As, Bs);
}

constexpr int SKS = 32;
constexpr int SPA = SKS + 1;
constexpr int SPB = NB + 32;
struct Tile32 {
  const gbyte* a;
  const gbyte* b;
  gfloat* out;
  int np, ke0, ke1;
  bool a64, b64, accumulate, negate;
};
__device__ __forceinline__ void tile32(const Tile32& o, float* __restrict__ As, float* __restrict__ Bs) {
  const int np = o.np;
  const int tid = threadIdx.x, lane = tid & 63, wave = tid >> 6, wm = wave >> 1, wn = wave & 1;
  const int l32 = lane & 31, h = lane >> 5;
  const long long a_off = (long long)(tid >> 3) * np + 4 * (tid & 7), a_step = 32ll * np;
  const long long b_off = (long long)(tid >> 4) * np + 4 * (tid & 15), b_step = 16ll * np;
  typedef const __attribute__((address_space(1))) f32x4 gf4;
  typedef const __attribute__((address_space(1))) f64x4 gd4;
  f32x4 ra[2], rb[2];
  auto fetch = [&](int ke) __attribute__((always_inline)) {
    if (o.a64) {
#pragma unroll
      for (int u = 0; u < 2; ++u) {
        const f64x4 v = *(gd4*)(o.a + (a_off + u * a_step + ke) * 8);
        ra[u] = f32x4{(float)v[0], (float)v[1], (float)v[2], (float)v[3]};
      }
    } else {
#pragma unroll
      for (int u = 0; u < 2; ++u) ra[u] = *(gf4*)(o.a + (a_off + u * a_step + ke) * 4);
    }
    if (o.b64) {
#pragma unroll
      for (int u = 0; u < 2; ++u) {
        const f64x4 v = *(gd4*)(o.b + (b_off + u * b_step + (long long)ke * np) * 8);
        rb[u] = f32x4{(float)v[0], (float)v[1], (float)v[2], (float)v[3]};
      }
    } else {
#pragma unroll
      for (int u = 0; u < 2; ++u) rb[u] = *(gf4*)(o.b + (b_off + u * b_step + (long long)ke * np) * 4);
    }
  };
  f32x16 acc = {0};
  fetch(o.ke0);
  for (int ke = o.ke0; ke < o.ke1; ke += SKS) {
#pragma unroll
    for (int u = 0; u < 2; ++u)
#pragma unroll
      for (int e = 0; e < 4; ++e) {
        As[((tid >> 3) + 32 * u) * SPA + 4 * (tid & 7) + e] = ra[u][e];
        Bs[((tid >> 4) + 16 * u) * SPB + 4 * (tid & 15) + e] = rb[u][e];
      }
    __syncthreads();
    if (ke + SKS < o.ke1) fetch(ke + SKS);
#pragma unroll
    for (int kk = 0; kk < SKS; kk += 2) {
      const float av = As[(32 * wm + l32) * SPA + kk + h];
      const float bv = Bs[(kk + h) * SPB + 32 * wn + l32];
      acc = __builtin_amdgcn_mfma_f32_32x32x2f32(av, bv, acc, 0, 0, 0);
    }
    __syncthreads();
  }
  gbyte* base = (gbyte*)(o.out + (long long)(32 * wm + 4 * h) * np + 32 * wn + l32);
  if (!o.accumulate) {
#pragma unroll
    for (int reg = 0; reg < 16; ++reg)
      *(gfloat*)(base + (long long)((reg & 3) + 8 * (reg >> 2)) * np * 4) = o.negate ? -acc[reg] : acc[reg];
  } else {
    float old[16];
#pragma unroll
    for (int reg = 0; reg < 16; ++reg) old[reg] = *(const gfloat*)(base + (long long)((reg & 3) + 8 * (reg >> 2)) * np * 4);
#pragma unroll
    for (int reg = 0; reg < 16; ++reg) *(gfloat*)(base + (long long)((reg & 3) + 8 * (reg >> 2)) * np * 4) = old[reg] + acc[reg];
  }
}
__device__ __host__ __forceinline__ long long supd_tiles(int P, int kind, int kend) {
  if (kind != 0 || P <= kend) return 0;
  const long long nsb = (P - kend + SB - 1) / SB, ncb = (kend + SB - 1) / SB;
  return nsb * ncb * (SB * SB);
}
__global__ void __launch_bounds__(INV_THREADS, 3)
supd32_kernel(const InvDev* __restrict__ t, int nf, int k0, int kend, int n_items) {
  __shared__ float As[NB * SPA], Bs[SKS * SPB];
  int item;
  {
    const int bid = blockIdx.x, xcd = bid & 7, jj = bid >> 3;
    item = ((jj / (SB * SB)) * 8 + xcd) * (SB * SB) + (jj % (SB * SB));
  }
  if (item >= n_items) return;
  int f, local;
  if (!locate(t, nf, item, [kend](const InvDev& d) { return (int)supd_tiles(d.P, s_kind(d), kend); }, f, local)) return;
  const InvDev& d = t[f];
  const int np = d.np, r = d.P - kend;
  const int ncb = (kend + SB - 1) / SB;
  const int sb = local / (SB * SB), in = local - sb * (SB * SB);
  const int a = sb / ncb, cb = sb - a * ncb;
  const int ri = a * SB + in / SB, j = cb * SB + in % SB;
  if (ri >= r || j >= kend) return;
  const int i = kend + ri;
  const bool own = j >= k0;
  Tile32 o;
  o.np = np;
  o.a = (const gbyte*)((const gfloat*)d.C32 + (long long)i * NB * np);
  o.a64 = false;
  o.b = own ? (const gbyte*)((const gdouble*)d.X + j * NB) : (const gbyte*)((const gfloat*)d.X32 + j * NB);
  o.b64 = own;
  o.ke0 = (own ? j : k0) * NB;
  o.ke1 = kend * NB;
  o.out = (gfloat*)d.S32 + (long long)i * NB * np + j * NB;
  o.accumulate = !own;
  o.negate = false;
  tile32(o, As, Bs);
}
__device__ __host__ __forceinline__ long long xrow_tiles(int P, int kind, int k0, int kend) {
  if (kind != 0 || P <= k0) return 0;
  return (long long)((kend < P ? kend : P) - k0) * k0;
}
__global__ void __launch_bounds__(INV_THREADS, 3)
xrows32_kernel(const InvDev* __restrict__ t, int nf, int k0, int kend) {
  __shared__ float As[NB * SPA], Bs[SKS * SPB];
  int f, local;
  if (!locate(t, nf, blockIdx.x, [k0, kend](const InvDev& d) { return (int)xrow_tiles(d.P, s_kind(d), k0, kend); }, f, local)) return;
  const InvDev& d = t[f];
  const int np = d.np, nb = (kend < d.P ? kend : d.P) - k0;
  const int j = local / nb, c = nb - 1 - (local - j * nb);
  Tile32 o;
  o.np = np;
  o.a = (const gbyte*)((const gdouble*)d.X + (long long)(k0 + c) * NB * np);
  o.a64 = true;
  o.b = (const gbyte*)((const gfloat*)d.S32 + j * NB);
  o.b64 = false;
  o.ke0 = k0 * NB;
  o.ke1 = (k0 + c + 1) * NB;
  o.out = (gfloat*)d.X32 + (long long)(k0 + c) * NB * np + j * NB;
  o.accumulate = false;
  o.negate = true;
  tile32(o, As, Bs);
}

__global__ void __launch_bounds__(INV_THREADS)
inv_finalize_kernel(const InvDev* __restrict__ t, int nf, int sq) {
  __shared__ float tile[NB][NB + 1];
  int f, local;
  if (!locate(t, nf, blockIdx.x, [](const InvDev& d) { return d.P * d.P; }, f, local)) return;
  const InvDev& d = t[f];
  const int n = d.n, np = d.np, q = d.P;
  const int ti = local / q, tj = local - ti * q;
  const gdouble* X = (const gdouble*)d.X;
  const gfloat* X32 = (const gfloat*)d.X32;
  gfloat* L = (gfloat*)d.L;
  const int w = __builtin_amdgcn_readfirstlane(threadIdx.x >> 6), c = threadIdx.x & 63;
  if (!d.reverse) {
    gdouble* Xo = (gdouble*)d.Xout;
    const gdouble* S = d.Zm != nullptr ? (const gdouble*)d.Zm : X;
#pragma unroll 4
    for (int u = 0; u < 16; ++u) {
      const int i = ti * NB + w + 4 * u, j = tj * NB + c;
      if (i < n && j < n) {
        double v = (j <= i) ? S[(long long)i * np + j] : 0.0;
        if (d.r_minus && j <= i) v = ((const gdouble*)d.R)[(long long)i * n + j] - v;
        Xo[(long long)i * n + j] = v;
      }
    }
    return;
  }
  if (tj > ti) {
#pragma unroll 4
    for (int u = 0; u < 16; ++u) {
      const int i = ti * NB + w + 4 * u, j = tj * NB + c;
      if (i < n && j < n) L[(long long)i * n + j] = 0.0f;
    }
    return;
  }
  double xv[16];
  const int i_l = ti * NB + c;
#pragma unroll
  for (int u = 0; u < 16; ++u) {
    const int j = tj * NB + w + 4 * u;
    const int rs = n - 1 - j, cs = n - 1 - i_l;
    const bool live = i_l < n && j < n && j <= i_l;
    if (X32 == nullptr || rs / sq == cs / sq) xv[u] = live ? X[(long long)rs * np + cs] : 0.0;
    else xv[u] = live ? (double)X32[(long long)rs * np + cs] : 0.0;
  }
#pragma unroll
  for (int u = 0; u < 16; ++u) tile[w + 4 * u][c] = (float)xv[u];
  __syncthreads();
#pragma unroll
  for (int u = 0; u < 16; ++u) {
    const int i = ti * NB + w + 4 * u, j = tj * NB + c;
    if (i < n && j < n) L[(long long)i * n + j] = tile[c][w + 4 * u];
  }
}

constexpr int INV_UPLOAD_CHUNK = 28;
static_assert(sizeof(InvDev) * INV_UPLOAD_CHUNK <= 3840, "a new InvDev field needs a hole in the row or a smaller chunk");

static size_t inv_table_bytes(int n) { return align_up((size_t)std::max(n, 1) * sizeof(InvDev), 256); }
static size_t inv_flags_bytes(int n) { return align_up((size_t)std::max(n, 1) * SQ_FLAGS * sizeof(int), 256); }

struct SideStream {
  hipStream_t stream = nullptr;
  hipEvent_t ev_main[2] = {nullptr, nullptr};
  hipEvent_t ev_side[2] = {nullptr, nullptr};
  hipEvent_t ev_tail = nullptr;
};
struct StreamSet {
  SideStream side[2];
  hipStream_t aux = nullptr;
  hipStream_t masked = nullptr;
  hipEvent_t ev_fork = nullptr, ev_join = nullptr, ev_join2 = nullptr;
  hipEvent_t ev_chain[2] = {nullptr, nullptr};
};
static std::mutex g_masked_mutex;
static std::vector<std::pair<int, hipStream_t>> g_masked_streams;
static void destroy_masked_streams() {
  std::lock_guard<std::mutex> lock(g_masked_mutex);
  for (auto& e : g_masked_streams) {
    if (hipSetDevice(e.first) == hipSuccess) {
      (void)hipStreamSynchronize(e.second);
      (void)hipStreamDestroy(e.second);
    }
  }
  g_masked_streams.clear();
}

static int stream_set(StreamSet** out) {
  static thread_local std::vector<std::pair<int, StreamSet>> cache;
  int dev = 0;
  CURV_HIP_CHECK(hipGetDevice(&dev));
  for (auto& e : cache) if (e.first == dev) { *out = &e.second; return CURV_OK; }
  StreamSet s;
  int prio_low = 0, prio_high = 0;
  CURV_HIP_CHECK(hipDeviceGetStreamPriorityRange(&prio_low, &prio_high));
  CURV_HIP_CHECK(hipEventCreateWithFlags(&s.ev_fork, hipEventDisableTiming));
  CURV_HIP_CHECK(hipEventCreateWithFlags(&s.ev_join, hipEventDisableTiming));
  CURV_HIP_CHECK(hipEventCreateWithFlags(&s.ev_join2, hipEventDisableTiming));
  for (int g = 0; g < 2; ++g) CURV_HIP_CHECK(hipEventCreateWithFlags(&s.ev_chain[g], hipEventDisableTiming));
  auto wide_stream = [&](hipStream_t* out) -> int {
    static const int free_cus = getenv("CURV_FREE_CUS") ? atoi(getenv("CURV_FREE_CUS")) : 32;
    hipDeviceProp_t prop;
    int dev_id = 0;
    CURV_HIP_CHECK(hipGetDevice(&dev_id));
    CURV_HIP_CHECK(hipGetDeviceProperties(&prop, dev_id));
    const int n_cu = prop.multiProcessorCount;
    if (free_cus > 0 && 2 * free_cus <= n_cu) {
      std::vector<uint32_t> mask((size_t)cdiv(n_cu, 32), 0u);
      for (int c = 0; c < n_cu - free_cus; ++c) mask[c >> 5] |= 1u << (c & 31);
      if (hipExtStreamCreateWithCUMask(out, (uint32_t)mask.size(), mask.data()) == hipSuccess) {
        std::lock_guard<std::mutex> lock(g_masked_mutex);
        if (g_masked_streams.empty()) atexit(destroy_masked_streams);
        g_masked_streams.emplace_back(dev_id, *out);
        return CURV_OK;
      }
      (void)hipGetLastError();
    }
    CURV_HIP_CHECK(hipStreamCreateWithPriority(out, hipStreamNonBlocking, prio_low));
    return CURV_OK;
  };
  CURV_HIP_CHECK(hipStreamCreateWithPriority(&s.aux, hipStreamNonBlocking, prio_high));
  CURV_HIP_CHECK(hipStreamCreateWithFlags(&s.masked, hipStreamNonBlocking));
  for (int g = 0; g < 2; ++g) {
    { const int rc = wide_stream(&s.side[g].stream); if (rc != CURV_OK) return rc; }
    for (int i = 0; i < 2; ++i) {
      CURV_HIP_CHECK(hipEventCreateWithFlags(&s.side[g].ev_main[i], hipEventDisableTiming));
      CURV_HIP_CHECK(hipEventCreateWithFlags(&s.side[g].ev_side[i], hipEventDisableTiming));
    }
    CURV_HIP_CHECK(hipEventCreateWithFlags(&s.side[g].ev_tail, hipEventDisableTiming));
  }
  cache.emplace_back(dev, s);
  *out = &cache.back().second;
  return CURV_OK;
}

int curv_internal_side_stream(hipStream_t* out) {
  StreamSet* ss = nullptr;
  const int rc = stream_set(&ss);
  if (rc != CURV_OK) return rc;
  *out = ss->masked;
  return CURV_OK;
}

}

using namespace curv;

#ifdef CURV_SQ_TRACE
extern "C" int curv_debug_sq_trace_reset() {
  long long zeros[256] = {0};
  return hipMemcpyToSymbol(HIP_SYMBOL(curv::g_sq_trace), zeros, sizeof(zeros)) == hipSuccess ? 0 : 1;
}
extern "C" int curv_debug_sq_trace(long long* out) {
  return hipMemcpyFromSymbol(out, HIP_SYMBOL(curv::g_sq_trace), 256 * sizeof(long long)) == hipSuccess ? 0 : 1;
}
#endif

extern "C" int curv_init_streams(void) {
  StreamSet* ss = nullptr;
  return stream_set(&ss);
}

extern "C" size_t curv_chol_inv_workspace_bytes(const curv_inv_desc* descs, int n_factors) {
  size_t total = 2 * inv_table_bytes(n_factors) + 2 * inv_flags_bytes(n_factors);
  for (int i = 0; i < n_factors; ++i) {
    if (descs[i].n <= 0) return 0;
    const size_t np = (size_t)cdiv(descs[i].n, NB) * NB;
    total += 2 * np * np * sizeof(double) + 3 * np * np * sizeof(float);
  }
  return total;
}

static int sweep_nbo(bool latency_bound) { return latency_bound ? 4 : 6; }
struct GroupSweep {
  hipStream_t stream;
  SideStream* side;
  const std::vector<InvDev>* tabp;
  InvDev* table;
  int* flags;
  bool latency_bound;
  int n_factors = 0, Pmax = 0, NBO = 4, k0 = 0, panel = 0;
  long long fin_tiles = 0, quarter_prod = 0;
  bool use_square = false, far_pending = false, inv_pending = false, capturing = false;

  GroupSweep(hipStream_t st, SideStream* sd, const std::vector<InvDev>& tab, InvDev* tb, int* fl, bool lb)
      : stream(st), side(sd), tabp(&tab), table(tb), flags(fl), latency_bound(lb) {}
  bool done() const { return k0 >= Pmax; }
  int panels() const { return cdiv(Pmax, NBO); }

  int begin() {
    const std::vector<InvDev>& tab = *tabp;
    n_factors = (int)tab.size();
    hipStreamCaptureStatus cap = hipStreamCaptureStatusNone;
    CURV_HIP_CHECK(hipStreamIsCapturing(stream, &cap));
    capturing = cap != hipStreamCaptureStatusNone;
    long long prep_tiles = 0;
    for (const InvDev& d : tab) {
      Pmax = std::max(Pmax, d.P);
      prep_tiles += (long long)d.P * (d.P + 1) / 2;
      fin_tiles += (long long)d.P * d.P;
    }
    const int rcu = upload_table<INV_UPLOAD_CHUNK>(stream, table, tab.data(), n_factors);
    if (rcu != CURV_OK) return rcu;
    hipLaunchKernelGGL(inv_prepare_kernel, dim3((unsigned)prep_tiles), dim3(INV_THREADS), 0, stream, table, n_factors, flags);
    CURV_LAUNCH_CHECK();
    NBO = sweep_nbo(latency_bound);
    return CURV_OK;
  }

  int panel_step() {
    const std::vector<InvDev>& tab = *tabp;
    constexpr long long WIDE_NEAR = 512, WIDE_PROD = 256;
    constexpr long long QUARTER_PROD = 512;
    quarter_prod = latency_bound ? QUARTER_PROD : 0;
    use_square = latency_bound;
    const int kend = k0 + NBO, row0 = kend + NBO;
    long long prod_tiles = 0;
    if (use_square) {
      long long sq_wgs = 0;
      for (const InvDev& d : tab)
        if (d.P > k0) sq_wgs += std::min(kend, d.P) - k0;
      hipLaunchKernelGGL(chol_square_kernel, dim3((unsigned)sq_wgs), dim3(INV_THREADS), 0, stream, table, n_factors, k0, kend,
                         flags, panel + 1);
      CURV_LAUNCH_CHECK();
    }
    for (int k = k0; !use_square && k < std::min(kend, Pmax); ++k) {
      long long diag_tiles = 0, panel_tiles = 0, upd_tiles = 0;
      for (const InvDev& d : tab) {
        if (d.P > k) { ++diag_tiles; panel_tiles += std::min(kend, d.P) - k0 - 1; }
        upd_tiles += inner_tiles(d.P, k, k0, kend);
      }
      if (k == k0) {
        hipLaunchKernelGGL(chol_diag_kernel, dim3((unsigned)diag_tiles), dim3(INV_THREADS), 0, stream, table, n_factors, k);
        CURV_LAUNCH_CHECK();
      }
      if (panel_tiles > 0) {
        hipLaunchKernelGGL(chol_panel_kernel, dim3((unsigned)panel_tiles), dim3(INV_THREADS), 0, stream, table, n_factors, k, k0, kend);
        CURV_LAUNCH_CHECK();
      }
      if (upd_tiles > 0) {
        hipLaunchKernelGGL(inner_update_kernel, dim3((unsigned)upd_tiles), dim3(INV_THREADS), 0, stream, table, n_factors, k, k0, kend);
        CURV_LAUNCH_CHECK();
      }
    }
    auto launch_product = [&](hipStream_t st, long long jobs, hipEvent_t done) -> int {
      const InvDev* tb = table;
      if (jobs <= quarter_prod)
        hipExtLaunchKernelGGL(panel_product_quarter_kernel, dim3((unsigned)(cdivll(jobs, 8) * 32)), dim3(INV_THREADS), 0, st,
                              nullptr, done, 0, tb, n_factors, k0, kend);
      else if (jobs <= WIDE_PROD)
        hipExtLaunchKernelGGL(panel_product_wide_kernel, dim3((unsigned)jobs), dim3(1024), 0, st, nullptr, done, 0, tb, n_factors,
                              k0, kend);
      else
        hipExtLaunchKernelGGL(panel_product_kernel, dim3((unsigned)jobs), dim3(INV_THREADS), 0, st, nullptr, done, 0, tb,
                              n_factors, k0, kend);
      CURV_LAUNCH_CHECK();
      return CURV_OK;
    };
    long long inv_jobs = 0, inv_tiles = 0;
    for (const InvDev& d : tab) {
      prod_tiles += panel_jobs(d.P, s_kind(d), k0, kend);
      inv_jobs += xrow_tiles(d.P, s_kind(d), k0, kend);
      inv_tiles += supd_tiles(d.P, s_kind(d), kend);
    }
    bool fork_recorded = false;
    if (prod_tiles > 0) {
      fork_recorded = !capturing;
      const int rc = launch_product(stream, prod_tiles, fork_recorded ? side->ev_main[panel & 1] : nullptr);
      if (rc != CURV_OK) return rc;
    }
    long long near_tiles = 0, far_tiles = 0;
    for (const InvDev& d : tab) {
      near_tiles += strip_tiles(d.P, kend, kend, row0, s_in_sweep(d));
      far_tiles += outer_tiles(d.P, kend, row0, s_in_sweep(d));
    }
    hipStream_t inv_st = side->stream;
    const bool inv_work = inv_jobs > 0 || inv_tiles > 0;
    const bool side_work = far_tiles > 0 || inv_work;
    if (side_work) {
      if (!fork_recorded) CURV_HIP_CHECK(hipEventRecord(side->ev_main[panel & 1], stream));
      CURV_HIP_CHECK(hipStreamWaitEvent(side->stream, side->ev_main[panel & 1], 0));
    }
    if (near_tiles > 0) {
      if (far_pending) {
        CURV_HIP_CHECK(hipStreamWaitEvent(stream, side->ev_side[(panel + 1) & 1], 0));
      }
      far_pending = false;
      if (near_tiles <= WIDE_NEAR)
        hipLaunchKernelGGL(outer_update_wide_kernel, dim3((unsigned)near_tiles), dim3(1024), 0, stream, table, n_factors,
                           k0, kend, kend, row0, 1, (int)near_tiles);
      else
        hipLaunchKernelGGL(outer_update_kernel, dim3((unsigned)near_tiles), dim3(INV_THREADS), 0, stream, table, n_factors, k0,
                           kend, kend, row0, 1, (int)near_tiles);
      CURV_LAUNCH_CHECK();
    }
    if (far_tiles > 0) {
      const bool ride = !capturing;
      const InvDev* tb = table;
      long long trail = 0;
      for (const InvDev& d : tab) trail += outer_tiles(d.P, kend, row0, false);
      const long long s_tiles = far_tiles - trail;
      if (trail > 0) {
        const long long g1 = cdivll(trail, 8 * SB * SB) * 8 * SB * SB;
        hipExtLaunchKernelGGL(outer_update_dma_kernel, dim3((unsigned)g1), dim3(INV_THREADS), 0, side->stream, nullptr,
                              (ride && s_tiles == 0) ? side->ev_side[panel & 1] : nullptr, 0, tb, n_factors, k0, kend, row0, (int)trail);
        CURV_LAUNCH_CHECK();
      }
      if (s_tiles > 0) {
        const long long g2 = cdivll(s_tiles, 8 * SB * SB) * 8 * SB * SB;
        hipExtLaunchKernelGGL(outer_update_kernel, dim3((unsigned)g2), dim3(INV_THREADS), 0, side->stream, nullptr,
                              ride ? side->ev_side[panel & 1] : nullptr, 0, tb, n_factors, k0, kend, row0, 0, 2, (int)s_tiles);
        CURV_LAUNCH_CHECK();
      }
      if (!ride) CURV_HIP_CHECK(hipEventRecord(side->ev_side[panel & 1], side->stream));
      far_pending = true;
    }
    if (inv_jobs > 0) {
      hipLaunchKernelGGL(xrows32_kernel, dim3((unsigned)inv_jobs), dim3(INV_THREADS), 0, inv_st, table, n_factors, k0, kend);
      CURV_LAUNCH_CHECK();
      inv_pending = true;
    }
    if (inv_tiles > 0) {
      const long long grid = cdivll(inv_tiles, 8 * SB * SB) * 8 * SB * SB;
      hipLaunchKernelGGL(supd32_kernel, dim3((unsigned)grid), dim3(INV_THREADS), 0, inv_st, table, n_factors, k0, kend,
                         (int)inv_tiles);
      CURV_LAUNCH_CHECK();
      inv_pending = true;
    }
    k0 += NBO;
    ++panel;
    return CURV_OK;
  }

  int end(hipEvent_t chain_done = nullptr) {
    if (chain_done != nullptr) CURV_HIP_CHECK(hipEventRecord(chain_done, stream));
    if (far_pending) CURV_HIP_CHECK(hipStreamWaitEvent(stream, side->ev_side[(panel + 1) & 1], 0));
    if (inv_pending) {
      CURV_HIP_CHECK(hipEventRecord(side->ev_tail, side->stream));
      CURV_HIP_CHECK(hipStreamWaitEvent(stream, side->ev_tail, 0));
    }
    hipLaunchKernelGGL(inv_finalize_kernel, dim3((unsigned)fin_tiles), dim3(INV_THREADS), 0, stream, table, n_factors, NBO * NB);
    CURV_LAUNCH_CHECK();
    return CURV_OK;
  }
};

static int chol_sweep_group(hipStream_t stream, SideStream* side, const std::vector<InvDev>& tab, InvDev* table, int* flags,
                            bool latency_bound, hipEvent_t chain_done = nullptr) {
  GroupSweep g(stream, side, tab, table, flags, latency_bound);
  int rc = g.begin();
  while (rc == CURV_OK && !g.done()) rc = g.panel_step();
  return rc == CURV_OK ? g.end(chain_done) : rc;
}

constexpr int SPLIT_P = 16;

struct EarlyStatus { int* host; const int* dev; size_t bytes; hipEvent_t ev; };

static int await_verdict(const EarlyStatus* early) {
  if (early != nullptr) CURV_HIP_CHECK(hipEventSynchronize(early->ev));
  return CURV_OK;
}

static int chol_sweep(hipStream_t stream, std::vector<InvDev>& tab, void* workspace, size_t workspace_bytes,
                      const char* who, const EarlyStatus* early = nullptr) {
  const int n_factors = (int)tab.size();
  static const int latency_max = getenv("CURV_LATENCY_MAX") ? atoi(getenv("CURV_LATENCY_MAX")) : 64;
  bool any_rhs = false;
  for (const InvDev& d : tab) any_rhs = any_rhs || d.R != nullptr;
  const bool latency_bound = n_factors <= latency_max && !any_rhs;
  size_t need = 2 * inv_table_bytes(n_factors) + 2 * inv_flags_bytes(n_factors);
  for (const InvDev& d : tab)
    need += (d.R != nullptr ? 3 : 2) * (size_t)d.np * d.np * sizeof(double) + (d.reverse ? 3 * (size_t)d.np * d.np * sizeof(float) : 0);
  if (workspace == nullptr || workspace_bytes < need) {
    set_error("%s: workspace too small (%zu < %zu bytes)", who, workspace_bytes, need);
    return CURV_ERR_WORKSPACE;
  }
  char* p = reinterpret_cast<char*>(workspace) + 2 * inv_table_bytes(n_factors);
  int* flags0 = reinterpret_cast<int*>(p);
  int* flags1 = reinterpret_cast<int*>(p + inv_flags_bytes(n_factors));
  p += 2 * inv_flags_bytes(n_factors);
  std::vector<InvDev> big, small;
  int Pmax = 0;
  for (const InvDev& d : tab) Pmax = std::max(Pmax, d.P);
  const int split = std::max(SPLIT_P, Pmax / 2);
  for (InvDev& d : tab) {
    d.W = reinterpret_cast<double*>(p); p += (size_t)d.np * d.np * sizeof(double);
    d.X = reinterpret_cast<double*>(p); p += (size_t)d.np * d.np * sizeof(double);
    if (d.R != nullptr) { d.Zm = reinterpret_cast<double*>(p); p += (size_t)d.np * d.np * sizeof(double); }
    if (d.reverse) {
      d.C32 = reinterpret_cast<float*>(p); p += (size_t)d.np * d.np * sizeof(float);
      d.X32 = reinterpret_cast<float*>(p); p += (size_t)d.np * d.np * sizeof(float);
      d.S32 = reinterpret_cast<float*>(p); p += (size_t)d.np * d.np * sizeof(float);
    }
    (d.P > split || latency_bound ? big : small).push_back(d);
  }
  StreamSet* ss = nullptr;
  { const int rc = stream_set(&ss); if (rc != CURV_OK) return rc; }
  InvDev* table0 = reinterpret_cast<InvDev*>(workspace);
  InvDev* table1 = reinterpret_cast<InvDev*>(reinterpret_cast<char*>(workspace) + inv_table_bytes(n_factors));
  hipStreamCaptureStatus capture = hipStreamCaptureStatusNone;
  CURV_HIP_CHECK(hipStreamIsCapturing(stream, &capture));
  if (capture != hipStreamCaptureStatusNone) {
    if (early != nullptr) {
      set_error("%s: the early status read-back is a host copy and cannot be captured", who);
      return CURV_ERR_INVALID;
    }
    if (!big.empty()) {
      const int rc = chol_sweep_group(stream, &ss->side[0], big, table0, flags0, latency_bound);
      if (rc != CURV_OK) return rc;
    }
    if (!small.empty()) return chol_sweep_group(stream, &ss->side[1], small, big.empty() ? table0 : table1,
                                                big.empty() ? flags0 : flags1, latency_bound);
    return CURV_OK;
  }
  if (big.empty() || small.empty()) {
    CURV_HIP_CHECK(hipEventRecord(ss->ev_fork, stream));
    CURV_HIP_CHECK(hipStreamWaitEvent(ss->aux, ss->ev_fork, 0));
    const int rc1 = chol_sweep_group(ss->aux, &ss->side[0], big.empty() ? small : big, table0, flags0, latency_bound,
                                     early ? ss->ev_chain[0] : nullptr);
    if (rc1 != CURV_OK) return rc1;
    if (early != nullptr) {
      CURV_HIP_CHECK(hipStreamWaitEvent(ss->side[0].stream, ss->ev_chain[0], 0));
      CURV_HIP_CHECK(hipMemcpyAsync(early->host, early->dev, early->bytes, hipMemcpyDeviceToHost, ss->side[0].stream));
      CURV_HIP_CHECK(hipEventRecord(early->ev, ss->side[0].stream));
    }
    { const int rc = await_verdict(early); if (rc != CURV_OK) return rc; }
    CURV_HIP_CHECK(hipEventRecord(ss->ev_join, ss->aux));
    CURV_HIP_CHECK(hipStreamWaitEvent(stream, ss->ev_join, 0));
    return CURV_OK;
  }
  CURV_HIP_CHECK(hipEventRecord(ss->ev_fork, stream));
  CURV_HIP_CHECK(hipStreamWaitEvent(ss->aux, ss->ev_fork, 0));
  CURV_HIP_CHECK(hipStreamWaitEvent(ss->masked, ss->ev_fork, 0));
  constexpr int START_FRAC = 30;
  const int n_panels = cdiv(Pmax, sweep_nbo(latency_bound));
  long long far0 = 0;
  for (const InvDev& d : big) far0 += outer_tiles(d.P, 4, 8, s_in_sweep(d));
  const int start_panel = far0 >= 5000 ? std::min(n_panels - 1, n_panels * START_FRAC / 100) : 0;
  GroupSweep gb(ss->aux, &ss->side[0], big, table0, flags0, latency_bound);
  GroupSweep gs(ss->masked, &ss->side[1], small, table1, flags1, latency_bound);
  int rc = gb.begin();
  if (rc != CURV_OK) return rc;
  bool small_started = false;
  for (int t = 0; !gb.done() || !small_started || !gs.done(); ++t) {
    if (!small_started && (t >= start_panel || gb.done())) {
      if (t > 0) {
        CURV_HIP_CHECK(hipEventRecord(ss->ev_join2, ss->aux));
        CURV_HIP_CHECK(hipStreamWaitEvent(ss->masked, ss->ev_join2, 0));
      }
      rc = gs.begin();
      if (rc != CURV_OK) return rc;
      small_started = true;
    }
    if (!gb.done()) { rc = gb.panel_step(); if (rc != CURV_OK) return rc; }
    if (small_started && !gs.done()) { rc = gs.panel_step(); if (rc != CURV_OK) return rc; }
  }
  rc = gb.end(early ? ss->ev_chain[0] : nullptr);
  if (rc != CURV_OK) return rc;
  rc = gs.end(early ? ss->ev_chain[1] : nullptr);
  if (rc != CURV_OK) return rc;
  if (early != nullptr) {
    CURV_HIP_CHECK(hipStreamWaitEvent(ss->side[1].stream, ss->ev_chain[0], 0));
    CURV_HIP_CHECK(hipStreamWaitEvent(ss->side[1].stream, ss->ev_chain[1], 0));
    CURV_HIP_CHECK(hipMemcpyAsync(early->host, early->dev, early->bytes, hipMemcpyDeviceToHost, ss->side[1].stream));
    CURV_HIP_CHECK(hipEventRecord(early->ev, ss->side[1].stream));
  }
  { const int rc = await_verdict(early); if (rc != CURV_OK) return rc; }
  CURV_HIP_CHECK(hipEventRecord(ss->ev_join, ss->aux));
  CURV_HIP_CHECK(hipStreamWaitEvent(stream, ss->ev_join, 0));
  CURV_HIP_CHECK(hipEventRecord(ss->ev_join2, ss->masked));
  CURV_HIP_CHECK(hipStreamWaitEvent(stream, ss->ev_join2, 0));
  return CURV_OK;
}

static int chol_inv_lower_impl(void* stream_, const curv_inv_desc* descs, int n_factors, int* info,
                               void* workspace, size_t workspace_bytes, const EarlyStatus* early);

constexpr int INV_MAX_N = 1 << 21;

extern "C" int curv_chol_inv_lower(void* stream_, const curv_inv_desc* descs, int n_factors, int* info,
                                   void* workspace, size_t workspace_bytes) {
  return chol_inv_lower_impl(stream_, descs, n_factors, info, workspace, workspace_bytes, nullptr);
}

extern "C" int curv_chol_inv_lower_status(void* stream_, const curv_inv_desc* descs, int n_factors, int* info,
                                          void* workspace, size_t workspace_bytes, int* host_status, void* ev_status) {
  CURV_REQUIRE(host_status != nullptr && ev_status != nullptr, "curv_chol_inv_lower_status: null argument");
  if (n_factors == 0) return CURV_OK;
  EarlyStatus early{host_status, info, (size_t)n_factors * sizeof(int), (hipEvent_t)ev_status};
  return chol_inv_lower_impl(stream_, descs, n_factors, info, workspace, workspace_bytes, &early);
}

static int chol_inv_lower_impl(void* stream_, const curv_inv_desc* descs, int n_factors, int* info,
                               void* workspace, size_t workspace_bytes, const EarlyStatus* early) {
  if (n_factors == 0) return CURV_OK;
  CURV_REQUIRE(descs != nullptr && info != nullptr, "curv_chol_inv_lower: null argument");
  std::vector<InvDev> tab(n_factors);
  for (int i = 0; i < n_factors; ++i) {
    const curv_inv_desc& s = descs[i];
    CURV_REQUIRE(s.n > 0, "curv_chol_inv_lower: factor %d: empty", i);
    CURV_REQUIRE(s.n <= INV_MAX_N, "curv_chol_inv_lower: factor %d: %d wide, the sweep takes at most %d", i, s.n, INV_MAX_N);
    CURV_REQUIRE(s.F != nullptr && s.L != nullptr, "curv_chol_inv_lower: factor %d: null pointer", i);
    CURV_REQUIRE(s.multiply >= 0.0 && s.add >= 0.0, "curv_chol_inv_lower: factor %d: negative hyper-parameter", i);
    InvDev& d = tab[i];
    memset(&d, 0, sizeof(d));
    d.F = s.F; d.L = s.L; d.n = s.n;
    d.P = cdiv(s.n, NB); d.np = d.P * NB;
    d.info = info + i;
    d.sqrt_s = (float)sqrt(s.multiply);
    d.sqrt_n = (float)sqrt(s.add);
    d.reverse = 1;
  }
  return chol_sweep((hipStream_t)stream_, tab, workspace, workspace_bytes, "curv_chol_inv_lower", early);
}

extern "C" size_t curv_chol_factor_inverse_workspace_bytes(const curv_cholinv_desc* descs, int n) {
  size_t total = 2 * inv_table_bytes(n) + 2 * inv_flags_bytes(n);
  for (int i = 0; i < n; ++i) {
    if (descs[i].n <= 0) return 0;
    const size_t np = (size_t)cdiv(descs[i].n, NB) * NB;
    total += (descs[i].R != nullptr ? 3 : 2) * np * np * sizeof(double);
  }
  return total;
}

extern "C" int curv_chol_factor_inverse(void* stream_, const curv_cholinv_desc* descs, int n_mats, int* info,
                                        void* workspace, size_t workspace_bytes) {
  if (n_mats == 0) return CURV_OK;
  CURV_REQUIRE(descs != nullptr && info != nullptr, "curv_chol_factor_inverse: null argument");
  std::vector<InvDev> tab(n_mats);
  for (int i = 0; i < n_mats; ++i) {
    const curv_cholinv_desc& s = descs[i];
    CURV_REQUIRE(s.n <= INV_MAX_N, "curv_chol_factor_inverse: matrix %d: %d wide, the sweep takes at most %d", i, s.n,
                 INV_MAX_N);
    CURV_REQUIRE(s.n > 0 && s.M != nullptr && s.X != nullptr, "curv_chol_factor_inverse: matrix %d invalid", i);
    InvDev& d = tab[i];
    memset(&d, 0, sizeof(d));
    d.F = reinterpret_cast<const float*>(s.M); d.Xout = s.X; d.n = s.n;
    d.f64_in = s.m_is_f64 ? 1 : 0;
    d.P = cdiv(s.n, NB); d.np = d.P * NB;
    d.info = info + i;
    d.sqrt_s = 1.0f;
    d.sqrt_n = (float)s.diag_add;
    d.add64 = s.diag_add;
    d.reverse = 0;
    d.pivot_min = s.pivot_min > 0.0 ? s.pivot_min : 0.0;
    d.R = s.R;
    d.r_minus = (s.R != nullptr && s.r_minus) ? 1 : 0;
  }
  return chol_sweep((hipStream_t)stream_, tab, workspace, workspace_bytes, "curv_chol_factor_inverse");
}
```

### curvature_amd/csrc/mma64.h

```cpp
#pragma once
#include "common.h"

namespace curv {

constexpr int NB = 64;
constexpr int MMA_THREADS = 256;
constexpr int LDA = NB + 1;

typedef __attribute__((address_space(1))) double gdouble;

template <bool BT>
__device__ __forceinline__ void mma_64(const double* __restrict__ As, const double* __restrict__ Bs, int wm,
                                       int wn, int lane, f64x4 (&acc)[2][2]) {
  const int r16 = lane & 15, kq = lane >> 4;
#pragma unroll 4
  for (int ks = 0; ks < NB / 4; ++ks) {
    const int k = 4 * ks + kq;
    double a[2], b[2];
#pragma unroll
    for (int m = 0; m < 2; ++m) a[m] = As[(32 * wm + 16 * m + r16) * LDA + k];
#pragma unroll
    for (int n = 0; n < 2; ++n)
      b[n] = BT ? Bs[(32 * wn + 16 * n + r16) * LDA + k] : Bs[k * LDA + 32 * wn + 16 * n + r16];
#pragma unroll
    for (int m = 0; m < 2; ++m)
#pragma unroll
      for (int n = 0; n < 2; ++n) acc[m][n] = __builtin_amdgcn_mfma_f64_16x16x4f64(a[m], b[n], acc[m][n], 0, 0, 0);
  }
}

typedef __attribute__((address_space(1))) char gbyte;
__device__ __forceinline__ void load_block(const gdouble* __restrict__ g, int ld, double* __restrict__ s) {
  const int tid = threadIdx.x, r0 = tid >> 6, c = tid & 63;
  const unsigned voff = (unsigned)(((long long)r0 * ld + c) * 8);
  const long long step = 4ll * ld * 8;
  const gbyte* base = (const gbyte*)g;
  double v[NB * NB / MMA_THREADS];
#pragma unroll
  for (int u = 0; u < NB * NB / MMA_THREADS; ++u) v[u] = *(const gdouble*)(base + u * step + voff);
#pragma unroll
  for (int u = 0; u < NB * NB / MMA_THREADS; ++u) s[(r0 + 4 * u) * LDA + c] = v[u];
}

__device__ __forceinline__ void store_block(gdouble* __restrict__ g, int ld, const double* __restrict__ s) {
  const int tid = threadIdx.x, r0 = tid >> 6, c = tid & 63;
  const unsigned voff = (unsigned)(((long long)r0 * ld + c) * 8);
  const long long step = 4ll * ld * 8;
  gbyte* base = (gbyte*)g;
#pragma unroll
  for (int u = 0; u < NB * NB / MMA_THREADS; ++u) *(gdouble*)(base + u * step + voff) = s[(r0 + 4 * u) * LDA + c];
}

__device__ __forceinline__ void store_acc(gdouble* __restrict__ C, int ld, const f64x4 (&acc)[2][2], int wm, int wn,
                                          int lane, int mode) {
  const int c16 = lane & 15, rq = lane >> 4;
  const unsigned voff = (unsigned)(((long long)(32 * wm + rq) * ld + 32 * wn + c16) * 8);
  gbyte* base = (gbyte*)C;
  double old[2][2][4];
  if (mode == 0 || mode == 2) {
#pragma unroll
    for (int m = 0; m < 2; ++m)
#pragma unroll
      for (int n = 0; n < 2; ++n)
#pragma unroll
        for (int q = 0; q < 4; ++q)
          old[m][n][q] = *(const gdouble*)(base + ((long long)(16 * m + 4 * q) * ld + 16 * n) * 8 + voff);
  }
#pragma unroll
  for (int m = 0; m < 2; ++m)
#pragma unroll
    for (int n = 0; n < 2; ++n)
#pragma unroll
      for (int q = 0; q < 4; ++q) {
        const double v = acc[m][n][q];
        const double out = mode == 0 ? old[m][n][q] - v : mode == 1 ? v : mode == 2 ? old[m][n][q] + v : -v;
        *(gdouble*)(base + ((long long)(16 * m + 4 * q) * ld + 16 * n) * 8 + voff) = out;
      }
}

__device__ __forceinline__ void acc_to_lds(const f64x4 (&acc)[2][2], int wm, int wn, int lane, double* s) {
  const int c16 = lane & 15, rq = lane >> 4;
#pragma unroll
  for (int m = 0; m < 2; ++m)
#pragma unroll
    for (int n = 0; n < 2; ++n)
#pragma unroll
      for (int r = 0; r < 4; ++r) s[(32 * wm + 16 * m + rq + 4 * r) * LDA + 32 * wn + 16 * n + c16] = acc[m][n][r];
}

}
```

Before: 4178.

## Pass small factor tables by value in kernel args and prefetch next diagonal block

All inversion sweep kernels are templated on a source type, so when a group has at most eight factors the InvDev descriptors travel inside the kernel argument block. The kernels then read their rows from arguments instead of a device table. This removes the global-memory table lookups and the scan in locate from every block. Separately, the inner update kernel loads the next diagonal block into registers before the MMA, overlapping that load with compute, at the cost of extra register pressure. A debug hook controls the by-value threshold.

```diff
diff --git a/curvature_amd/_lib.py b/curvature_amd/_lib.py
--- a/curvature_amd/_lib.py
+++ b/curvature_amd/_lib.py
@@ -464,6 +464,11 @@
 ERR_NOT_PD, ERR_INVALID, ERR_WORKSPACE, ERR_HIP, ERR_NOT_CONVERGED = 1, 2, 3, 4, 5
 
 
+INTERNAL = {
+    "curv_debug_inv_by_value_max": (_i, [_i]),
+}
+
+
 def lib() -> ctypes.CDLL:
     global _lib
     if _lib is not None:
@@ -477,7 +482,7 @@
                 f"{LIB_PATH} is missing: run `python -c 'import __graft_entry__ as g; g.build()'` "
                 "(hipcc --offload-arch=gfx950). There is no CPU fallback.")
         handle = ctypes.CDLL(LIB_PATH, mode=ctypes.RTLD_GLOBAL)
-        for name, (res, args) in SIGNATURES.items():
+        for name, (res, args) in list(SIGNATURES.items()) + list(INTERNAL.items()):
             fn = getattr(handle, name)
             fn.restype = res
             fn.argtypes = args
diff --git a/curvature_amd/csrc/invert.hip b/curvature_amd/csrc/invert.hip
--- a/curvature_amd/csrc/invert.hip
+++ b/curvature_amd/csrc/invert.hip
@@ -4,6 +4,7 @@
 #include <hip/hip_ext.h>
 
 #include <algorithm>
+#include <atomic>
 #include <chrono>
 #include <cstdlib>
 #include <mutex>
@@ -84,11 +85,57 @@
   return false;
 }
 
+constexpr int INV_BY_VALUE = 8;
+struct InvEntry {
+  InvDev d;
+  int base;
+  int slot;
+};
+using InvArgs = ArgBatch<InvEntry, INV_BY_VALUE>;
+static_assert(sizeof(InvArgs) + 64 <= 3840, "kernel argument block (the batch and the launch's scalars) must stay below 4 KB");
+
+static std::atomic<int> g_by_value_max{INV_BY_VALUE};
+
+struct FromTable {
+  const InvDev* t;
+  int nf;
+  template <typename CountFn>
+  __device__ __forceinline__ bool find(int unit, CountFn cnt, int& f, int& local) const {
+    return locate(t, nf, unit, cnt, f, local);
+  }
+  __device__ __forceinline__ const InvDev& row(int f) const { return t[f]; }
+  __device__ __forceinline__ int slot(int f) const { return f; }
+};
+struct ByValue {
+  InvArgs b;
+  template <typename CountFn>
+  __device__ __forceinline__ bool find(int unit, CountFn cnt, int& f, int& local) const {
+    f = owner_of_early_exit(b, unit);
+    local = unit - b.e[f].base;
+    return local < cnt(b.e[f].d);
+  }
+  __device__ __forceinline__ const InvDev& row(int f) const { return b.e[f].d; }
+  __device__ __forceinline__ int slot(int f) const { return b.e[f].slot; }
+};
+
+struct CntPrepare { __device__ __host__ int operator()(const InvDev& d) const { return d.P * (d.P + 1) / 2; } };
+struct CntFinalize { __device__ __host__ int operator()(const InvDev& d) const { return d.P * d.P; } };
+struct CntDiag { int k; __device__ __host__ int operator()(const InvDev& d) const { return d.P > k ? 1 : 0; } };
+struct CntPanel {
+  int k, k0, kend;
+  __device__ __host__ int operator()(const InvDev& d) const { return d.P > k ? (kend < d.P ? kend : d.P) - k0 - 1 : 0; }
+};
+struct CntSquare {
+  int k0, kend;
+  __device__ __host__ int operator()(const InvDev& d) const { return d.P > k0 ? (kend < d.P ? kend : d.P) - k0 : 0; }
+};
+
+template <typename Src>
 __global__ void __launch_bounds__(INV_THREADS)
-inv_prepare_kernel(const InvDev* __restrict__ t, int nf, int* __restrict__ flags) {
+inv_prepare_kernel(const Src src, int* __restrict__ flags) {
   int f, tile;
-  if (!locate(t, nf, blockIdx.x, [](const InvDev& d) { return d.P * (d.P + 1) / 2; }, f, tile)) return;
-  const InvDev& d = t[f];
+  if (!src.find(blockIdx.x, CntPrepare{}, f, tile)) return;
+  const InvDev& d = src.row(f);
   int bi = 0;
   while (tile > bi) { tile -= bi + 1; ++bi; }
   const int bj = tile;
@@ -97,7 +144,7 @@
   const gfloat* F = (const gfloat*)d.F;
   gdouble* W = (gdouble*)d.W;
   if (bi == 0 && bj == 0 && threadIdx.x == 0) *d.info = 0;
-  if (bi == 0 && bj == 0 && threadIdx.x < SQ_FLAGS) flags[(long long)f * SQ_FLAGS + threadIdx.x] = 0;
+  if (bi == 0 && bj == 0 && threadIdx.x < SQ_FLAGS) flags[(long long)src.slot(f) * SQ_FLAGS + threadIdx.x] = 0;
   if (d.Zm != nullptr) {
     const gdouble* Rg = (const gdouble*)d.R;
     gdouble* Z = (gdouble*)d.Zm;
@@ -182,6 +229,25 @@
   return n;
 }
 
+struct CntInner {
+  int k, k0, kend;
+  __device__ __host__ int operator()(const InvDev& d) const { return (int)inner_tiles(d.P, k, k0, kend); }
+};
+struct CntStrip {
+  int kend, lo, hi;
+  __device__ __host__ int operator()(const InvDev& d) const { return (int)strip_tiles(d.P, kend, lo, hi, s_in_sweep(d)); }
+};
+struct CntFarS {
+  int kend, row0;
+  __device__ __host__ int operator()(const InvDev& d) const {
+    return (int)(outer_tiles(d.P, kend, row0, s_in_sweep(d)) - outer_tiles(d.P, kend, row0, false));
+  }
+};
+struct CntFarTrail {
+  int kend, row0;
+  __device__ __host__ int operator()(const InvDev& d) const { return (int)outer_tiles(d.P, kend, row0, false); }
+};
+
 __device__ __forceinline__ void store_sub(gdouble* C, int np, const f64x4 (&acc)[2][2], int wm, int wn, int lane,
                                           int mode) {
   store_acc(C, np, acc, wm, wn, lane, mode);
@@ -190,12 +256,13 @@
 __device__ __forceinline__ void factor_invert_64(double* Ds, double* Is, int* bad, int pivot_base, double pivot_min, int trace_base = -1);
 __device__ __forceinline__ void lds_sub_acc(double* s, const f64x4 (&acc)[2][2], int wm, int wn, int lane);
 
+template <typename Src>
 __global__ void __launch_bounds__(INV_THREADS)
-inner_update_kernel(const InvDev* __restrict__ t, int nf, int k, int k0, int kend) {
+inner_update_kernel(const Src src, int k, int k0, int kend) {
   __shared__ double As[NB * LDA], Bs[NB * LDA];
   int f, local;
-  if (!locate(t, nf, blockIdx.x, [k, k0, kend](const InvDev& d) { return (int)inner_tiles(d.P, k, k0, kend); }, f, local)) return;
-  const InvDev& d = t[f];
+  if (!src.find(blockIdx.x, CntInner{k, k0, kend}, f, local)) return;
+  const InvDev& d = src.row(f);
   const int np = d.np, P = d.P, ke = kend < P ? kend : P;
   gdouble* W = (gdouble*)d.W;
   gdouble* X = (gdouble*)d.X;
@@ -209,15 +276,18 @@
   }
   if (trailing) {
     const int i = j + local;
+    const bool next_diag = i == j && j == k + 1;
     load_block(W + (long long)i * NB * np + k * NB, np, As);
     if (i != j) load_block(W + (long long)j * NB * np + k * NB, np, Bs);
+    double ajj[NB * NB / MMA_THREADS];
+    if (next_diag) fetch_block(W + (long long)j * NB * np + j * NB, np, ajj);
     __syncthreads();
     mma_64<true>(As, (i != j) ? Bs : As, wm, wn, lane, acc);
-    if (i == j && j == k + 1) {
+    if (next_diag) {
       __shared__ int bad;
       __syncthreads();
       if (threadIdx.x == 0) bad = 0;
-      load_block(W + (long long)j * NB * np + j * NB, np, As);
+      put_block(ajj, As);
       __syncthreads();
       {
         const int c16 = lane & 15, rq = lane >> 4;
@@ -357,15 +427,14 @@
   else tile_product_impl<WV, 0>(o, As, Bs);
 }
 
-template <int WV>
-__device__ __forceinline__ void outer_update_body(const InvDev* __restrict__ t, int nf, int k0, int kend, int lo, int hi,
+template <int WV, typename Src>
+__device__ __forceinline__ void outer_update_body(const Src& src, int k0, int kend, int lo, int hi,
                                                   int strip, int n_items, double* __restrict__ As, double* __restrict__ Bs) {
   bool trailing;
   int i, j, f, local;
   if (strip == 1) {
-    if (!locate(t, nf, blockIdx.x, [kend, lo, hi](const InvDev& d) { return (int)strip_tiles(d.P, kend, lo, hi, s_in_sweep(d)); }, f, local))
-      return;
-    const int P = t[f].P, re = hi < P ? hi : P;
+    if (!src.find(blockIdx.x, CntStrip{kend, lo, hi}, f, local)) return;
+    const int P = src.row(f).P, re = hi < P ? hi : P;
     trailing = false;
     j = lo;
     for (; j < re; ++j) {
@@ -386,9 +455,8 @@
       item = ((jj / (SB * SB)) * 8 + xcd) * (SB * SB) + (jj % (SB * SB));
     }
     if (item >= n_items) return;
-    if (!locate(t, nf, item, [kend, row0](const InvDev& d) {
-          return (int)(outer_tiles(d.P, kend, row0, s_in_sweep(d)) - outer_tiles(d.P, kend, row0, false)); }, f, local)) return;
-    const int r = t[f].P - row0;
+    if (!src.find(item, CntFarS{kend, row0}, f, local)) return;
+    const int r = src.row(f).P - row0;
     const int s2 = local / (SB * SB), in = local % (SB * SB);
     const int di = in / SB, dj = in - di * SB;
     const int ncb = (kend + SB - 1) / SB;
@@ -397,7 +465,7 @@
     if (ri >= r || j >= kend) return;
     trailing = false; i = row0 + ri;
   }
-  const InvDev& d = t[f];
+  const InvDev& d = src.row(f);
   const int np = d.np;
   const gdouble* W = (const gdouble*)d.W;
   gdouble* X = (gdouble*)d.X;
@@ -414,10 +482,11 @@
   o.mode = trailing ? 0 : (d.Zm != nullptr ? 0 : (j >= k0 ? 1 : 2));
   tile_product_k32<WV>(o, As, Bs);
 }
+template <typename Src>
 __global__ void __launch_bounds__(INV_THREADS, 3)
-outer_update_kernel(const InvDev* __restrict__ t, int nf, int k0, int kend, int lo, int hi, int strip, int n_items) {
+outer_update_kernel(const Src src, int k0, int kend, int lo, int hi, int strip, int n_items) {
   __shared__ double As[NB * OPA], Bs[NB * OPA > OKS * LDA ? NB * OPA : OKS * LDA];
-  outer_update_body<2>(t, nf, k0, kend, lo, hi, strip, n_items, As, Bs);
+  outer_update_body<2>(src, k0, kend, lo, hi, strip, n_items, As, Bs);
 }
 typedef __attribute__((address_space(3))) void lds_void;
 typedef __attribute__((address_space(3))) char lds_char;
@@ -425,8 +494,9 @@
 namespace fard {
 constexpr int ROW_B = 128, TILE_B = NB * ROW_B, KS = 16;
 }
+template <typename Src>
 __global__ void __launch_bounds__(INV_THREADS, 4)
-outer_update_dma_kernel(const InvDev* __restrict__ t, int nf, int k0, int kend, int row0, int n_items) {
+outer_update_dma_kernel(const Src src, int k0, int kend, int row0, int n_items) {
   using namespace fard;
   __shared__ __attribute__((aligned(1024))) char smem[4 * TILE_B];
   lds_char* lds = (lds_char*)smem;
@@ -437,8 +507,8 @@
   }
   if (item >= n_items) return;
   int f, local;
-  if (!locate(t, nf, item, [kend, row0](const InvDev& d) { return (int)outer_tiles(d.P, kend, row0, false); }, f, local)) return;
-  const InvDev& d = t[f];
+  if (!src.find(item, CntFarTrail{kend, row0}, f, local)) return;
+  const InvDev& d = src.row(f);
   int i, j;
   {
     const int r = d.P - row0;
@@ -507,11 +577,12 @@
   store_acc((gdouble*)d.W + (long long)i * NB * np + j * NB, np, acc, wm, wn, lane, 0);
 }
 
+template <typename Src>
 __global__ void __launch_bounds__(1024)
-outer_update_wide_kernel(const InvDev* __restrict__ t, int nf, int k0, int kend, int lo, int hi, int strip, int n_items) {
+outer_update_wide_kernel(const Src src, int k0, int kend, int lo, int hi, int strip, int n_items) {
   __shared__ double As[NB * OPA], Bs[NB * OPA > OKS * LDA ? NB * OPA : OKS * LDA];
   KT_BEGIN(252)
-  outer_update_body<4>(t, nf, k0, kend, lo, hi, strip, n_items, As, Bs);
+  outer_update_body<4>(src, k0, kend, lo, hi, strip, n_items, As, Bs);
   KT_END(253)
 }
 
@@ -688,14 +759,15 @@
   __syncthreads();
 }
 
+template <typename Src>
 __global__ void __launch_bounds__(INV_THREADS)
-chol_diag_kernel(const InvDev* __restrict__ t, int nf, int k) {
+chol_diag_kernel(const Src src, int k) {
   __shared__ double Ds[NB * LDA];
   __shared__ double Is[NB * LDA];
   __shared__ int bad;
   int f, local;
-  if (!locate(t, nf, blockIdx.x, [k](const InvDev& d) { return d.P > k ? 1 : 0; }, f, local)) return;
-  const InvDev& d = t[f];
+  if (!src.find(blockIdx.x, CntDiag{k}, f, local)) return;
+  const InvDev& d = src.row(f);
   const int np = d.np, tid = threadIdx.x;
   gdouble* W = (gdouble*)d.W;
   if (tid == 0) bad = 0;
@@ -706,14 +778,13 @@
   if (tid == 0 && bad != 0) atomicCAS(d.info, 0, bad);
 }
 
+template <typename Src>
 __global__ void __launch_bounds__(INV_THREADS)
-chol_panel_kernel(const InvDev* __restrict__ t, int nf, int k, int k0, int kend) {
+chol_panel_kernel(const Src src, int k, int k0, int kend) {
   __shared__ double As[NB * LDA], Bs[NB * LDA];
   int f, local;
-  if (!locate(t, nf, blockIdx.x,
-              [k, k0, kend](const InvDev& d) { return d.P > k ? (kend < d.P ? kend : d.P) - k0 - 1 : 0; }, f, local))
-    return;
-  const InvDev& d = t[f];
+  if (!src.find(blockIdx.x, CntPanel{k, k0, kend}, f, local)) return;
+  const InvDev& d = src.row(f);
   const int np = d.np, n_solve = (kend < d.P ? kend : d.P) - k - 1;
   gdouble* W = (gdouble*)d.W;
   gdouble* X = (gdouble*)d.X;
@@ -821,19 +892,19 @@
   __syncthreads();
 }
 
+template <typename Src>
 __global__ void __launch_bounds__(INV_THREADS)
-chol_square_kernel(const InvDev* __restrict__ t, int nf, int k0, int kend, int* __restrict__ flags, int stamp) {
+chol_square_kernel(const Src src, int k0, int kend, int* __restrict__ flags, int stamp) {
   __shared__ double Ds[NB * LDA], Is[NB * LDA], Bf[NB * LDA];
   __shared__ int bad, lost;
   int f, r;
-  if (!locate(t, nf, blockIdx.x, [k0, kend](const InvDev& d) { return d.P > k0 ? (kend < d.P ? kend : d.P) - k0 : 0; }, f, r))
-    return;
-  const InvDev& d = t[f];
+  if (!src.find(blockIdx.x, CntSquare{k0, kend}, f, r)) return;
+  const InvDev& d = src.row(f);
   const int np = d.np, tid = threadIdx.x;
   const int nbf = (kend < d.P ? kend : d.P) - k0;
   gdouble* W = (gdouble*)d.W;
   gdouble* X = (gdouble*)d.X;
-  int* fl = flags + (long long)f * SQ_FLAGS;
+  int* fl = flags + (long long)src.slot(f) * SQ_FLAGS;
   const int lane = tid & 63, wave = tid >> 6, wm = wave >> 1, wn = wave & 1;
   auto Wt = [&](int i, int j) { return W + (long long)(k0 + i) * NB * np + (k0 + j) * NB; };
   auto Xt = [&](int i, int j) { return X + (long long)(k0 + i) * NB * np + (k0 + j) * NB; };
@@ -975,13 +1046,16 @@
   if (P <= k0) return 0;
   return (P > kend ? P - kend : 0) + (kind == 2 ? (kend < P ? kend : P) : kind == 1 ? k0 : 0);
 }
-template <int WV>
-__device__ __forceinline__ void panel_product_body(const InvDev* __restrict__ t, int nf, int k0, int kend,
+struct CntProduct {
+  int k0, kend;
+  __device__ __host__ int operator()(const InvDev& d) const { return panel_jobs(d.P, s_kind(d), k0, kend); }
+};
+template <int WV, typename Src>
+__device__ __forceinline__ void panel_product_body(const Src& src, int k0, int kend,
                                                    double* __restrict__ As, double* __restrict__ Bs) {
   int f, local;
-  if (!locate(t, nf, blockIdx.x, [k0, kend](const InvDev& d) { return panel_jobs(d.P, s_kind(d), k0, kend); }, f, local))
-    return;
-  const InvDev& d = t[f];
+  if (!src.find(blockIdx.x, CntProduct{k0, kend}, f, local)) return;
+  const InvDev& d = src.row(f);
   const int np = d.np, nb = (kend < d.P ? kend : d.P) - k0;
   gdouble* W = (gdouble*)d.W;
   gdouble* X = (gdouble*)d.X;
@@ -1099,29 +1173,32 @@
     step(rt2);
   }
 }
+template <typename Src>
 __global__ void __launch_bounds__(INV_THREADS)
-panel_product_quarter_kernel(const InvDev* __restrict__ t, int nf, int k0, int kend) {
+panel_product_quarter_kernel(const Src src, int k0, int kend) {
   __shared__ double Own[PQ_OWN], Ts[NB * LDA];
   const int job = (blockIdx.x >> 5) * 8 + (blockIdx.x & 7), q = (blockIdx.x >> 3) & 3;
   int f, local;
   KT_BEGIN(236)
-  if (!locate(t, nf, job, [k0, kend](const InvDev& d) { return panel_jobs(d.P, s_kind(d), k0, kend); }, f, local)) return;
-  const InvDev& d = t[f];
+  if (!src.find(job, CntProduct{k0, kend}, f, local)) return;
+  const InvDev& d = src.row(f);
   const int nb = (kend < d.P ? kend : d.P) - k0;
   const int n_below = d.P > kend ? d.P - kend : 0;
   if (local < n_below) panel_quarter_body<true>(d, k0, nb, kend + local, 0, q, Own, Ts);
   else panel_quarter_body<false>(d, k0, nb, 0, local - n_below, q, Own, Ts);
   KT_END(237)
 }
+template <typename Src>
 __global__ void __launch_bounds__(INV_THREADS, 3)
-panel_product_kernel(const InvDev* __restrict__ t, int nf, int k0, int kend) {
+panel_product_kernel(const Src src, int k0, int kend) {
   __shared__ double As[NB * OPA], Bs[NB * OPA > OKS * LDA ? NB * OPA : OKS * LDA];
-  panel_product_body<2>(t, nf, k0, kend, As, Bs);
-}
+  panel_product_body<2>(src, k0, kend, As, Bs);
+}
+template <typename Src>
 __global__ void __launch_bounds__(1024)
-panel_product_wide_kernel(const InvDev* __restrict__ t, int nf, int k0, int kend) {
+panel_product_wide_kernel(const Src src, int k0, int kend) {
   __shared__ double As[NB * OPA], Bs[NB * OPA > OKS * LDA ? NB * OPA : OKS * LDA];
-  panel_product_body<4>(t, nf, k0, kend, As, Bs);
+  panel_product_body<4>(src, k0, kend, As, Bs);
 }
 
 constexpr int SKS = 32;
@@ -1203,8 +1280,13 @@
   const long long nsb = (P - kend + SB - 1) / SB, ncb = (kend + SB - 1) / SB;
   return nsb * ncb * (SB * SB);
 }
+struct CntSupd {
+  int kend;
+  __device__ __host__ int operator()(const InvDev& d) const { return (int)supd_tiles(d.P, s_kind(d), kend); }
+};
+template <typename Src>
 __global__ void __launch_bounds__(INV_THREADS, 3)
-supd32_kernel(const InvDev* __restrict__ t, int nf, int k0, int kend, int n_items) {
+supd32_kernel(const Src src, int k0, int kend, int n_items) {
   __shared__ float As[NB * SPA], Bs[SKS * SPB];
   int item;
   {
@@ -1213,8 +1295,8 @@
   }
   if (item >= n_items) return;
   int f, local;
-  if (!locate(t, nf, item, [kend](const InvDev& d) { return (int)supd_tiles(d.P, s_kind(d), kend); }, f, local)) return;
-  const InvDev& d = t[f];
+  if (!src.find(item, CntSupd{kend}, f, local)) return;
+  const InvDev& d = src.row(f);
   const int np = d.np, r = d.P - kend;
   const int ncb = (kend + SB - 1) / SB;
   const int sb = local / (SB * SB), in = local - sb * (SB * SB);
@@ -1240,12 +1322,17 @@
   if (kind != 0 || P <= k0) return 0;
   return (long long)((kend < P ? kend : P) - k0) * k0;
 }
+struct CntXrows {
+  int k0, kend;
+  __device__ __host__ int operator()(const InvDev& d) const { return (int)xrow_tiles(d.P, s_kind(d), k0, kend); }
+};
+template <typename Src>
 __global__ void __launch_bounds__(INV_THREADS, 3)
-xrows32_kernel(const InvDev* __restrict__ t, int nf, int k0, int kend) {
+xrows32_kernel(const Src src, int k0, int kend) {
   __shared__ float As[NB * SPA], Bs[SKS * SPB];
   int f, local;
-  if (!locate(t, nf, blockIdx.x, [k0, kend](const InvDev& d) { return (int)xrow_tiles(d.P, s_kind(d), k0, kend); }, f, local)) return;
-  const InvDev& d = t[f];
+  if (!src.find(blockIdx.x, CntXrows{k0, kend}, f, local)) return;
+  const InvDev& d = src.row(f);
   const int np = d.np, nb = (kend < d.P ? kend : d.P) - k0;
   const int j = local / nb, c = nb - 1 - (local - j * nb);
   Tile32 o;
@@ -1262,12 +1349,13 @@
   tile32(o, As, Bs);
 }
 
+template <typename Src>
 __global__ void __launch_bounds__(INV_THREADS)
-inv_finalize_kernel(const InvDev* __restrict__ t, int nf, int sq) {
+inv_finalize_kernel(const Src src, int sq) {
   __shared__ float tile[NB][NB + 1];
   int f, local;
-  if (!locate(t, nf, blockIdx.x, [](const InvDev& d) { return d.P * d.P; }, f, local)) return;
-  const InvDev& d = t[f];
+  if (!src.find(blockIdx.x, CntFinalize{}, f, local)) return;
+  const InvDev& d = src.row(f);
   const int n = d.n, np = d.np, q = d.P;
   const int ti = local / q, tj = local - ti * q;
   const gdouble* X = (const gdouble*)d.X;
@@ -1418,6 +1506,10 @@
 }
 #endif
 
+extern "C" int curv_debug_inv_by_value_max(int n) {
+  return g_by_value_max.exchange(n < 0 || n > INV_BY_VALUE ? INV_BY_VALUE : n);
+}
+
 extern "C" int curv_init_streams(void) {
   StreamSet* ss = nullptr;
   return stream_set(&ss);
@@ -1444,9 +1536,36 @@
   int n_factors = 0, Pmax = 0, NBO = 4, k0 = 0, panel = 0;
   long long fin_tiles = 0, quarter_prod = 0;
   bool use_square = false, far_pending = false, inv_pending = false, capturing = false;
-
-  GroupSweep(hipStream_t st, SideStream* sd, const std::vector<InvDev>& tab, InvDev* tb, int* fl, bool lb)
-      : stream(st), side(sd), tabp(&tab), table(tb), flags(fl), latency_bound(lb) {}
+  int by_value_max;
+
+  GroupSweep(hipStream_t st, SideStream* sd, const std::vector<InvDev>& tab, InvDev* tb, int* fl, bool lb, int by_value)
+      : stream(st), side(sd), tabp(&tab), table(tb), flags(fl), latency_bound(lb),
+        by_value_max(std::min(std::max(by_value, 0), INV_BY_VALUE)) {}
+
+  template <typename Cnt, typename Go>
+  int with_source(Cnt cnt, Go go) {
+    const std::vector<InvDev>& tab = *tabp;
+    ByValue v;
+    int n = 0;
+    long long units = 0;
+    bool fits = true;
+    for (size_t f = 0; f < tab.size(); ++f) {
+      const int c = cnt(tab[f]);
+      if (c <= 0) continue;
+      if (n == by_value_max) { fits = false; break; }
+      v.b.e[n].d = tab[f];
+      v.b.e[n].base = (int)units;
+      v.b.e[n].slot = (int)f;
+      units += c;
+      ++n;
+    }
+    if (!fits) return go(FromTable{table, n_factors});
+    if (n == 0) return CURV_OK;
+    CURV_REQUIRE(units < (1LL << 31), "inversion sweep: too many work items in one launch (%lld)", units);
+    v.b.count = n;
+    for (int k = n; k < INV_BY_VALUE; ++k) v.b.e[k] = v.b.e[0];
+    return go(v);
+  }
   bool done() const { return k0 >= Pmax; }
   int panels() const { return cdiv(Pmax, NBO); }
 
@@ -1462,10 +1581,19 @@
       prep_tiles += (long long)d.P * (d.P + 1) / 2;
       fin_tiles += (long long)d.P * d.P;
     }
-    const int rcu = upload_table<INV_UPLOAD_CHUNK>(stream, table, tab.data(), n_factors);
-    if (rcu != CURV_OK) return rcu;
-    hipLaunchKernelGGL(inv_prepare_kernel, dim3((unsigned)prep_tiles), dim3(INV_THREADS), 0, stream, table, n_factors, flags);
-    CURV_LAUNCH_CHECK();
+    if (n_factors > by_value_max) {
+      const int rcu = upload_table<INV_UPLOAD_CHUNK>(stream, table, tab.data(), n_factors);
+      if (rcu != CURV_OK) return rcu;
+    }
+    {
+      const int rc = with_source(CntPrepare{}, [&](const auto& src) -> int {
+        using Src = std::decay_t<decltype(src)>;
+        hipLaunchKernelGGL((inv_prepare_kernel<Src>), dim3((unsigned)prep_tiles), dim3(INV_THREADS), 0, stream, src, flags);
+        CURV_LAUNCH_CHECK();
+        return CURV_OK;
+      });
+      if (rc != CURV_OK) return rc;
+    }
     NBO = sweep_nbo(latency_bound);
     return CURV_OK;
   }
@@ -1482,9 +1610,14 @@
       long long sq_wgs = 0;
       for (const InvDev& d : tab)
         if (d.P > k0) sq_wgs += std::min(kend, d.P) - k0;
-      hipLaunchKernelGGL(chol_square_kernel, dim3((unsigned)sq_wgs), dim3(INV_THREADS), 0, stream, table, n_factors, k0, kend,
-                         flags, panel + 1);
-      CURV_LAUNCH_CHECK();
+      const int rc = with_source(CntSquare{k0, kend}, [&](const auto& src) -> int {
+        using Src = std::decay_t<decltype(src)>;
+        hipLaunchKernelGGL((chol_square_kernel<Src>), dim3((unsigned)sq_wgs), dim3(INV_THREADS), 0, stream, src, k0, kend, flags,
+                           panel + 1);
+        CURV_LAUNCH_CHECK();
+        return CURV_OK;
+      });
+      if (rc != CURV_OK) return rc;
     }
     for (int k = k0; !use_square && k < std::min(kend, Pmax); ++k) {
       long long diag_tiles = 0, panel_tiles = 0, upd_tiles = 0;
@@ -1492,32 +1625,48 @@
         if (d.P > k) { ++diag_tiles; panel_tiles += std::min(kend, d.P) - k0 - 1; }
         upd_tiles += inner_tiles(d.P, k, k0, kend);
       }
+      int rc = CURV_OK;
       if (k == k0) {
-        hipLaunchKernelGGL(chol_diag_kernel, dim3((unsigned)diag_tiles), dim3(INV_THREADS), 0, stream, table, n_factors, k);
+        rc = with_source(CntDiag{k}, [&](const auto& src) -> int {
+          using Src = std::decay_t<decltype(src)>;
+          hipLaunchKernelGGL((chol_diag_kernel<Src>), dim3((unsigned)diag_tiles), dim3(INV_THREADS), 0, stream, src, k);
+          CURV_LAUNCH_CHECK();
+          return CURV_OK;
+        });
+      }
+      if (rc == CURV_OK && panel_tiles > 0) {
+        rc = with_source(CntPanel{k, k0, kend}, [&](const auto& src) -> int {
+          using Src = std::decay_t<decltype(src)>;
+          hipLaunchKernelGGL((chol_panel_kernel<Src>), dim3((unsigned)panel_tiles), dim3(INV_THREADS), 0, stream, src, k, k0, kend);
+          CURV_LAUNCH_CHECK();
+          return CURV_OK;
+        });
+      }
+      if (rc == CURV_OK && upd_tiles > 0) {
+        rc = with_source(CntInner{k, k0, kend}, [&](const auto& src) -> int {
+          using Src = std::decay_t<decltype(src)>;
+          hipLaunchKernelGGL((inner_update_kernel<Src>), dim3((unsigned)upd_tiles), dim3(INV_THREADS), 0, stream, src, k, k0, kend);
+          CURV_LAUNCH_CHECK();
+          return CURV_OK;
+        });
+      }
+      if (rc != CURV_OK) return rc;
+    }
+    auto launch_product = [&](hipStream_t st, long long jobs, hipEvent_t done) -> int {
+      return with_source(CntProduct{k0, kend}, [&](const auto& src) -> int {
+        using Src = std::decay_t<decltype(src)>;
+        if (jobs <= quarter_prod)
+          hipExtLaunchKernelGGL((panel_product_quarter_kernel<Src>), dim3((unsigned)(cdivll(jobs, 8) * 32)), dim3(INV_THREADS), 0,
+                                st, nullptr, done, 0, src, k0, kend);
+        else if (jobs <= WIDE_PROD)
+          hipExtLaunchKernelGGL((panel_product_wide_kernel<Src>), dim3((unsigned)jobs), dim3(1024), 0, st, nullptr, done, 0, src,
+                                k0, kend);
+        else
+          hipExtLaunchKernelGGL((panel_product_kernel<Src>), dim3((unsigned)jobs), dim3(INV_THREADS), 0, st, nullptr, done, 0,
+                                src, k0, kend);
         CURV_LAUNCH_CHECK();
-      }
-      if (panel_tiles > 0) {
-        hipLaunchKernelGGL(chol_panel_kernel, dim3((unsigned)panel_tiles), dim3(INV_THREADS), 0, stream, table, n_factors, k, k0, kend);
-        CURV_LAUNCH_CHECK();
-      }
-      if (upd_tiles > 0) {
-        hipLaunchKernelGGL(inner_update_kernel, dim3((unsigned)upd_tiles), dim3(INV_THREADS), 0, stream, table, n_factors, k, k0, kend);
-        CURV_LAUNCH_CHECK();
-      }
-    }
-    auto launch_product = [&](hipStream_t st, long long jobs, hipEvent_t done) -> int {
-      const InvDev* tb = table;
-      if (jobs <= quarter_prod)
-        hipExtLaunchKernelGGL(panel_product_quarter_kernel, dim3((unsigned)(cdivll(jobs, 8) * 32)), dim3(INV_THREADS), 0, st,
-                              nullptr, done, 0, tb, n_factors, k0, kend);
-      else if (jobs <= WIDE_PROD)
-        hipExtLaunchKernelGGL(panel_product_wide_kernel, dim3((unsigned)jobs), dim3(1024), 0, st, nullptr, done, 0, tb, n_factors,
-                              k0, kend);
-      else
-        hipExtLaunchKernelGGL(panel_product_kernel, dim3((unsigned)jobs), dim3(INV_THREADS), 0, st, nullptr, done, 0, tb,
-                              n_factors, k0, kend);
-      CURV_LAUNCH_CHECK();
-      return CURV_OK;
+        return CURV_OK;
+      });
     };
     long long inv_jobs = 0, inv_tiles = 0;
     for (const InvDev& d : tab) {
@@ -1548,45 +1697,69 @@
         CURV_HIP_CHECK(hipStreamWaitEvent(stream, side->ev_side[(panel + 1) & 1], 0));
       }
       far_pending = false;
-      if (near_tiles <= WIDE_NEAR)
-        hipLaunchKernelGGL(outer_update_wide_kernel, dim3((unsigned)near_tiles), dim3(1024), 0, stream, table, n_factors,
-                           k0, kend, kend, row0, 1, (int)near_tiles);
-      else
-        hipLaunchKernelGGL(outer_update_kernel, dim3((unsigned)near_tiles), dim3(INV_THREADS), 0, stream, table, n_factors, k0,
-                           kend, kend, row0, 1, (int)near_tiles);
-      CURV_LAUNCH_CHECK();
+      const int rc = with_source(CntStrip{kend, kend, row0}, [&](const auto& src) -> int {
+        using Src = std::decay_t<decltype(src)>;
+        if (near_tiles <= WIDE_NEAR)
+          hipLaunchKernelGGL((outer_update_wide_kernel<Src>), dim3((unsigned)near_tiles), dim3(1024), 0, stream, src, k0, kend,
+                             kend, row0, 1, (int)near_tiles);
+        else
+          hipLaunchKernelGGL((outer_update_kernel<Src>), dim3((unsigned)near_tiles), dim3(INV_THREADS), 0, stream, src, k0, kend,
+                             kend, row0, 1, (int)near_tiles);
+        CURV_LAUNCH_CHECK();
+        return CURV_OK;
+      });
+      if (rc != CURV_OK) return rc;
     }
     if (far_tiles > 0) {
       const bool ride = !capturing;
-      const InvDev* tb = table;
       long long trail = 0;
       for (const InvDev& d : tab) trail += outer_tiles(d.P, kend, row0, false);
       const long long s_tiles = far_tiles - trail;
       if (trail > 0) {
         const long long g1 = cdivll(trail, 8 * SB * SB) * 8 * SB * SB;
-        hipExtLaunchKernelGGL(outer_update_dma_kernel, dim3((unsigned)g1), dim3(INV_THREADS), 0, side->stream, nullptr,
-                              (ride && s_tiles == 0) ? side->ev_side[panel & 1] : nullptr, 0, tb, n_factors, k0, kend, row0, (int)trail);
-        CURV_LAUNCH_CHECK();
+        const int rc = with_source(CntFarTrail{kend, row0}, [&](const auto& src) -> int {
+          using Src = std::decay_t<decltype(src)>;
+          hipExtLaunchKernelGGL((outer_update_dma_kernel<Src>), dim3((unsigned)g1), dim3(INV_THREADS), 0, side->stream, nullptr,
+                                (ride && s_tiles == 0) ? side->ev_side[panel & 1] : nullptr, 0, src, k0, kend, row0, (int)trail);
+          CURV_LAUNCH_CHECK();
+          return CURV_OK;
+        });
+        if (rc != CURV_OK) return rc;
       }
       if (s_tiles > 0) {
         const long long g2 = cdivll(s_tiles, 8 * SB * SB) * 8 * SB * SB;
-        hipExtLaunchKernelGGL(outer_update_kernel, dim3((unsigned)g2), dim3(INV_THREADS), 0, side->stream, nullptr,
-                              ride ? side->ev_side[panel & 1] : nullptr, 0, tb, n_factors, k0, kend, row0, 0, 2, (int)s_tiles);
-        CURV_LAUNCH_CHECK();
+        const int rc = with_source(CntFarS{kend, row0}, [&](const auto& src) -> int {
+          using Src = std::decay_t<decltype(src)>;
+          hipExtLaunchKernelGGL((outer_update_kernel<Src>), dim3((unsigned)g2), dim3(INV_THREADS), 0, side->stream, nullptr,
+                                ride ? side->ev_side[panel & 1] : nullptr, 0, src, k0, kend, row0, 0, 2, (int)s_tiles);
+          CURV_LAUNCH_CHECK();
+          return CURV_OK;
+        });
+        if (rc != CURV_OK) return rc;
       }
       if (!ride) CURV_HIP_CHECK(hipEventRecord(side->ev_side[panel & 1], side->stream));
       far_pending = true;
     }
     if (inv_jobs > 0) {
-      hipLaunchKernelGGL(xrows32_kernel, dim3((unsigned)inv_jobs), dim3(INV_THREADS), 0, inv_st, table, n_factors, k0, kend);
-      CURV_LAUNCH_CHECK();
+      const int rc = with_source(CntXrows{k0, kend}, [&](const auto& src) -> int {
+        using Src = std::decay_t<decltype(src)>;
+        hipLaunchKernelGGL((xrows32_kernel<Src>), dim3((unsigned)inv_jobs), dim3(INV_THREADS), 0, inv_st, src, k0, kend);
+        CURV_LAUNCH_CHECK();
+        return CURV_OK;
+      });
+      if (rc != CURV_OK) return rc;
       inv_pending = true;
     }
     if (inv_tiles > 0) {
       const long long grid = cdivll(inv_tiles, 8 * SB * SB) * 8 * SB * SB;
-      hipLaunchKernelGGL(supd32_kernel, dim3((unsigned)grid), dim3(INV_THREADS), 0, inv_st, table, n_factors, k0, kend,
-                         (int)inv_tiles);
-      CURV_LAUNCH_CHECK();
+      const int rc = with_source(CntSupd{kend}, [&](const auto& src) -> int {
+        using Src = std::decay_t<decltype(src)>;
+        hipLaunchKernelGGL((supd32_kernel<Src>), dim3((unsigned)grid), dim3(INV_THREADS), 0, inv_st, src, k0, kend,
+                           (int)inv_tiles);
+        CURV_LAUNCH_CHECK();
+        return CURV_OK;
+      });
+      if (rc != CURV_OK) return rc;
       inv_pending = true;
     }
     k0 += NBO;
@@ -1601,15 +1774,18 @@
       CURV_HIP_CHECK(hipEventRecord(side->ev_tail, side->stream));
       CURV_HIP_CHECK(hipStreamWaitEvent(stream, side->ev_tail, 0));
     }
-    hipLaunchKernelGGL(inv_finalize_kernel, dim3((unsigned)fin_tiles), dim3(INV_THREADS), 0, stream, table, n_factors, NBO * NB);
-    CURV_LAUNCH_CHECK();
-    return CURV_OK;
+    return with_source(CntFinalize{}, [&](const auto& src) -> int {
+      using Src = std::decay_t<decltype(src)>;
+      hipLaunchKernelGGL((inv_finalize_kernel<Src>), dim3((unsigned)fin_tiles), dim3(INV_THREADS), 0, stream, src, NBO * NB);
+      CURV_LAUNCH_CHECK();
+      return CURV_OK;
+    });
   }
 };
 
 static int chol_sweep_group(hipStream_t stream, SideStream* side, const std::vector<InvDev>& tab, InvDev* table, int* flags,
-                            bool latency_bound, hipEvent_t chain_done = nullptr) {
-  GroupSweep g(stream, side, tab, table, flags, latency_bound);
+                            bool latency_bound, int by_value, hipEvent_t chain_done = nullptr) {
+  GroupSweep g(stream, side, tab, table, flags, latency_bound, by_value);
   int rc = g.begin();
   while (rc == CURV_OK && !g.done()) rc = g.panel_step();
   return rc == CURV_OK ? g.end(chain_done) : rc;
@@ -1659,6 +1835,7 @@
   }
   StreamSet* ss = nullptr;
   { const int rc = stream_set(&ss); if (rc != CURV_OK) return rc; }
+  const int by_value = g_by_value_max.load();
   InvDev* table0 = reinterpret_cast<InvDev*>(workspace);
   InvDev* table1 = reinterpret_cast<InvDev*>(reinterpret_cast<char*>(workspace) + inv_table_bytes(n_factors));
   hipStreamCaptureStatus capture = hipStreamCaptureStatusNone;
@@ -1669,18 +1846,18 @@
       return CURV_ERR_INVALID;
     }
     if (!big.empty()) {
-      const int rc = chol_sweep_group(stream, &ss->side[0], big, table0, flags0, latency_bound);
+      const int rc = chol_sweep_group(stream, &ss->side[0], big, table0, flags0, latency_bound, by_value);
       if (rc != CURV_OK) return rc;
     }
     if (!small.empty()) return chol_sweep_group(stream, &ss->side[1], small, big.empty() ? table0 : table1,
-                                                big.empty() ? flags0 : flags1, latency_bound);
+                                                big.empty() ? flags0 : flags1, latency_bound, big.empty() ? by_value : 0);
     return CURV_OK;
   }
   if (big.empty() || small.empty()) {
     CURV_HIP_CHECK(hipEventRecord(ss->ev_fork, stream));
     CURV_HIP_CHECK(hipStreamWaitEvent(ss->aux, ss->ev_fork, 0));
     const int rc1 = chol_sweep_group(ss->aux, &ss->side[0], big.empty() ? small : big, table0, flags0, latency_bound,
-                                     early ? ss->ev_chain[0] : nullptr);
+                                     by_value, early ? ss->ev_chain[0] : nullptr);
     if (rc1 != CURV_OK) return rc1;
     if (early != nullptr) {
       CURV_HIP_CHECK(hipStreamWaitEvent(ss->side[0].stream, ss->ev_chain[0], 0));
@@ -1700,8 +1877,8 @@
   long long far0 = 0;
   for (const InvDev& d : big) far0 += outer_tiles(d.P, 4, 8, s_in_sweep(d));
   const int start_panel = far0 >= 5000 ? std::min(n_panels - 1, n_panels * START_FRAC / 100) : 0;
-  GroupSweep gb(ss->aux, &ss->side[0], big, table0, flags0, latency_bound);
-  GroupSweep gs(ss->masked, &ss->side[1], small, table1, flags1, latency_bound);
+  GroupSweep gb(ss->aux, &ss->side[0], big, table0, flags0, latency_bound, by_value);
+  GroupSweep gs(ss->masked, &ss->side[1], small, table1, flags1, latency_bound, 0);
   int rc = gb.begin();
   if (rc != CURV_OK) return rc;
   bool small_started = false;
diff --git a/curvature_amd/csrc/mma64.h b/curvature_amd/csrc/mma64.h
--- a/curvature_amd/csrc/mma64.h
+++ b/curvature_amd/csrc/mma64.h
@@ -38,6 +38,20 @@
   double v[NB * NB / MMA_THREADS];
 #pragma unroll
   for (int u = 0; u < NB * NB / MMA_THREADS; ++u) v[u] = *(const gdouble*)(base + u * step + voff);
+#pragma unroll
+  for (int u = 0; u < NB * NB / MMA_THREADS; ++u) s[(r0 + 4 * u) * LDA + c] = v[u];
+}
+
+__device__ __forceinline__ void fetch_block(const gdouble* __restrict__ g, int ld, double (&v)[NB * NB / MMA_THREADS]) {
+  const int tid = threadIdx.x, r0 = tid >> 6, c = tid & 63;
+  const unsigned voff = (unsigned)(((long long)r0 * ld + c) * 8);
+  const long long step = 4ll * ld * 8;
+  const gbyte* base = (const gbyte*)g;
+#pragma unroll
+  for (int u = 0; u < NB * NB / MMA_THREADS; ++u) v[u] = *(const gdouble*)(base + u * step + voff);
+}
+__device__ __forceinline__ void put_block(const double (&v)[NB * NB / MMA_THREADS], double* __restrict__ s) {
+  const int tid = threadIdx.x, r0 = tid >> 6, c = tid & 63;
 #pragma unroll
   for (int u = 0; u < NB * NB / MMA_THREADS; ++u) s[(r0 + 4 * u) * LDA + c] = v[u];
 }
```

Result: slower. 4136 (-1.0%).
